# samivout/clair-torch

Hardware: AMD Instinct MI355X
Metric: MPix/s HDR-merged (+uncertainty) at N=32 4K RGB (higher is better)
Workload: dtype f32; 1 GPU; C2: 32-exposure 4096x4096x3 uint16 stack per GPU, merge+uncertainty (LINEAR ICRF 3x256, Gaussian weights, sigma: multiplier, float64 mean + float32 std out); global_image=4096x4096x3 in 1 row band(s)

## Files before the change

clair_torch_amd/_native.py:

```python
import ctypes
import os

from . import build as _build

DTYPE_U8, DTYPE_U16, DTYPE_F32 = 0, 1, 2
INTERP_LOOKUP, INTERP_LINEAR, INTERP_CATMULL, INTERP_NONE = 0, 1, 2, 3
STD_NONE, STD_CONSTANT, STD_MULTIPLIER, STD_EXPLICIT = 0, 1, 2, 3
WEIGHT_NONE, WEIGHT_GAUSS = 0, 1
LAYOUT_NCHW, LAYOUT_NHWC, LAYOUT_NHWC_BGR = 0, 1, 2
MERGE_FIRST_BATCH, MERGE_FINALIZE, MERGE_MEAN_OUT_F32, MERGE_F64_MOMENTS = 1, 2, 4, 8
MERGE_REFERENCE_ORDER, MERGE_CLOSED_FORM, MERGE_STD_HINT, MERGE_REQUIRE_ONE_LAUNCH, MERGE_OUT_AS_INPUT = 16, 32, 64, 128, 256
INGEST_AFFINE, INGEST_CLAMP, INGEST_MAX_STAGES, INGEST_MAX_CHANNELS = 0, 1, 4, 4
INGEST_AFFINE_DATA, EXTREMA_MIN, EXTREMA_MAX, EXTREMA_MAX_PREFIX = 2, 1, 2, 3
ERR_NO_GRADIENT_PATH = -4

ABI_VERSION = 3
EXPORTS = ("ct_abi_version", "ct_error_string", "ct_hdr_merge_batch", "ct_hdr_merge_batches", "ct_linearize_std", "ct_linearize_fwd",
           "ct_linearize_bwd", "ct_pair_residual_fwd", "ct_pair_residual_bwd", "ct_pair_residual_bwd_workspace", "ct_flatfield_sums",
           "ct_flatfield_apply", "ct_video_stats_batch", "ct_dark_field_blur", "ct_hdr_merge_kernel_name",
           "ct_merge_set_retry_counter", "ct_norm_constants", "ct_index_constants", "ct_pivot_index_constants",
           "ct_pivot_floor_constants", "ct_pivot_interval_constants", "ct_band_stats", "ct_band_stats_workspace",
           "ct_strided_downscale", "ct_export_cv", "ct_ingest_transform", "ct_ingest_extrema_workspace", "ct_ingest_extrema",
           "ct_ingest_transform_data", "ct_linearize_ingest")


class Geometry(ctypes.Structure):
    _fields_ = [("channels", ctypes.c_int32), ("h_tile", ctypes.c_int64), ("width", ctypes.c_int64),
                ("h_global", ctypes.c_int64), ("row_offset", ctypes.c_int64), ("image_stride", ctypes.c_int64),
                ("layout", ctypes.c_int32)]


class Icrf(ctypes.Structure):
    _fields_ = [("lut_dev", ctypes.c_void_p), ("n_points", ctypes.c_int32), ("interp", ctypes.c_int32)]


class PairParams(ctypes.Structure):
    _fields_ = [("lower", ctypes.c_float), ("upper", ctypes.c_float), ("weight_scale", ctypes.c_float),
                ("use_relative", ctypes.c_int32), ("use_uncertainty_weighting", ctypes.c_int32),
                ("std_mode", ctypes.c_int32), ("std_value", ctypes.c_float), ("pair_band", ctypes.c_int32)]


class IngestStage(ctypes.Structure):
    _fields_ = [("kind", ctypes.c_int32), ("sub", ctypes.c_float), ("div", ctypes.c_float), ("mul", ctypes.c_float),
                ("add", ctypes.c_float), ("lo", ctypes.c_float * 4), ("hi", ctypes.c_float * 4)]


class NativeLibraryError(RuntimeError):
    pass


_lib = None


def library_path():
    return _build.LIB_PATH


def load():
    global _lib
    if _lib is not None:
        return _lib
    path = library_path()
    if not os.path.exists(path):
        raise NativeLibraryError(
            f"{path} is missing: build it with `python -m clair_torch_amd.build` (hipcc, gfx950). "
            "clair_torch_amd has no CPU fallback for its kernels.")
    lib = ctypes.CDLL(path)
    vp, i32, i64, f32, u32 = ctypes.c_void_p, ctypes.c_int32, ctypes.c_int64, ctypes.c_float, ctypes.c_uint32
    gp, ip = ctypes.POINTER(Geometry), ctypes.POINTER(Icrf)
    lib.ct_abi_version.restype = i32
    lib.ct_error_string.restype = ctypes.c_char_p
    lib.ct_error_string.argtypes = [i32]
    lib.ct_hdr_merge_batch.restype = i32
    lib.ct_hdr_merge_batch.argtypes = [vp, i32, f32, i32, gp, vp, i32, f32, vp, ip, i32, vp, vp, vp, vp, vp, u32, vp]
    lib.ct_hdr_merge_batches.restype = i32
    lib.ct_hdr_merge_batches.argtypes = [vp, vp, vp, i32, i32, f32, gp, i32, f32, vp, ip, i32, vp, vp, vp, vp, vp, u32, vp]
    lib.ct_pivot_interval_constants.restype = i32
    lib.ct_pivot_interval_constants.argtypes = [f32, i32, i32, i32, ctypes.POINTER(f32)]
    lib.ct_linearize_std.restype = i32
    lib.ct_linearize_std.argtypes = [vp, i32, f32, i64, gp, vp, i32, f32, ip, vp, vp, vp]
    lib.ct_linearize_fwd.restype = i32
    lib.ct_linearize_fwd.argtypes = [vp, i64, gp, ip, vp, vp]
    lib.ct_linearize_bwd.restype = i32
    lib.ct_linearize_bwd.argtypes = [vp, vp, i64, gp, ip, vp, vp, vp]
    pp = ctypes.POINTER(PairParams)
    lib.ct_pair_residual_fwd.restype = i32
    lib.ct_pair_residual_fwd.argtypes = [vp, i32, f32, i32, gp, vp, ip, vp, vp, vp, i32, pp, i32, vp, vp, vp]
    lib.ct_pair_residual_bwd.restype = i32
    lib.ct_pair_residual_bwd.argtypes = [vp, i32, f32, i32, gp, vp, ip, vp, i32, vp, vp, vp, pp, vp, vp, vp, vp, i64, vp]
    lib.ct_pair_residual_bwd_workspace.restype = i64
    lib.ct_pair_residual_bwd_workspace.argtypes = [i32, i32, i32]
    lib.ct_hdr_merge_kernel_name.restype = ctypes.c_char_p
    lib.ct_hdr_merge_kernel_name.argtypes = [i32, f32, i32, i32, u32]
    lib.ct_merge_set_retry_counter.restype = None
    lib.ct_merge_set_retry_counter.argtypes = [vp]
    lib.ct_flatfield_sums.restype = i32
    lib.ct_flatfield_sums.argtypes = [vp, i32, vp, i32, i64, vp, vp]
    lib.ct_flatfield_apply.restype = i32
    lib.ct_flatfield_apply.argtypes = [vp, i32, i64, vp, i32, vp, vp, vp, vp, i32, i64, vp]
    lib.ct_dark_field_blur.restype = i32
    lib.ct_dark_field_blur.argtypes = [vp, i32, f32, i32, gp, vp, vp, i32, f32, vp, vp, i32, f32, f32, vp, vp, vp]
    lib.ct_band_stats_workspace.restype = i64
    lib.ct_band_stats_workspace.argtypes = [i32]
    lib.ct_band_stats.restype = i32
    lib.ct_band_stats.argtypes = [vp, vp, i32, i64, vp, i64, vp, vp]
    lib.ct_strided_downscale.restype = i32
    lib.ct_strided_downscale.argtypes = [vp, vp, i32, i64, i64, i64, i32, i32, vp]
    lib.ct_export_cv.restype = i32
    lib.ct_export_cv.argtypes = [vp, i32, vp, i32, i64, i32, i64, i32, vp]
    lib.ct_ingest_transform.restype = i32
    lib.ct_ingest_transform.argtypes = [vp, i32, i32, i64, i32, i64, ctypes.POINTER(IngestStage), i32, vp, vp]
    lib.ct_ingest_extrema_workspace.restype = i64
    lib.ct_ingest_extrema_workspace.argtypes = []
    lib.ct_ingest_extrema.restype = i32
    lib.ct_ingest_extrema.argtypes = [vp, i32, i32, i64, i32, i64, ctypes.POINTER(IngestStage), i32, i32, f32, f32, vp, i64, vp, vp]
    lib.ct_ingest_transform_data.restype = i32
    lib.ct_ingest_transform_data.argtypes = [vp, i32, i32, i64, i32, i64, ctypes.POINTER(IngestStage), i32, vp, vp, vp]
    lib.ct_linearize_ingest.restype = i32
    lib.ct_linearize_ingest.argtypes = [vp, i32, i64, gp, ctypes.POINTER(IngestStage), i32, vp, i32, f32, ip, vp, vp, vp]
    lib.ct_video_stats_batch.restype = i32
    lib.ct_video_stats_batch.argtypes = [vp, i32, f32, i32, gp, ip, f32, vp, vp, vp]
    if lib.ct_abi_version() != ABI_VERSION:
        raise NativeLibraryError(f"{path}: ABI version {lib.ct_abi_version()} != {ABI_VERSION}; rebuild the library")
    _lib = lib
    return lib


def check(rc, what):
    if rc == 0:
        return
    msg = load().ct_error_string(rc).decode()
    if rc == ERR_NO_GRADIENT_PATH:
        raise RuntimeError("element 0 of tensors does not require grad and does not have a grad_fn")
    if rc in (-1, -5):
        raise ValueError(f"{what}: {msg}")
    raise NativeLibraryError(f"{what}: {msg} (code {rc})")
```

clair_torch_amd/build.py:

```python
import os
import shutil
import subprocess
import sys
from concurrent.futures import ThreadPoolExecutor

HERE = os.path.dirname(os.path.abspath(__file__))
CSRC = os.path.join(HERE, "csrc")
LIB_DIR = os.path.join(HERE, "lib")
LIB_PATH = os.path.join(LIB_DIR, "libclair_hip.so")
OBJ_DIR = os.path.join(LIB_DIR, "obj")
SOURCES = ["ct_merge.hip", "ct_merge_multi.hip", "ct_merge_exact.hip", "ct_linearize.hip", "ct_pairs.hip", "ct_flatfield.hip", "ct_stats.hip", "ct_darkfield.hip", "ct_bandstats.hip",
           "ct_downscale.hip", "ct_export.hip", "ct_ingest.hip", "ct_extrema.hip", "ct_linearize_ingest.hip", "ct_api.cpp"]
HEADERS = ["ct_device.hpp", "ct_merge.hpp", "ct_merge_pivot.hpp", "ct_ingest_stages.hpp", os.path.join("..", "..", "include", "clair_hip.h")]
FLAGS = ["--offload-arch=gfx950", "-O3", "-std=c++17", "-fPIC", "-ffp-contract=off",
         "-fno-slp-vectorize", "-Wall", "-Wno-unused-function", "-Wno-pass-failed"]


def _hipcc():
    for cand in (os.environ.get("HIPCC"), shutil.which("hipcc"), "/opt/rocm/bin/hipcc"):
        if cand and os.path.exists(cand):
            return cand
    raise RuntimeError("hipcc not found (set HIPCC or install ROCm under /opt/rocm)")


def is_stale():
    if not os.path.exists(LIB_PATH):
        return True
    built = os.path.getmtime(LIB_PATH)
    deps = [os.path.join(CSRC, s) for s in SOURCES if os.path.exists(os.path.join(CSRC, s))]
    deps += [os.path.join(CSRC, h) for h in HEADERS]
    return any(os.path.getmtime(d) > built for d in deps)


def _object_is_stale(src, obj):
    if not os.path.exists(obj):
        return True
    built = os.path.getmtime(obj)
    return any(os.path.getmtime(d) > built for d in [src] + [os.path.join(CSRC, h) for h in HEADERS])


def build(force=False, verbose=False):
    if not force and not is_stale():
        return LIB_PATH
    os.makedirs(OBJ_DIR, exist_ok=True)
    hipcc = _hipcc()
    srcs = [os.path.join(CSRC, s) for s in SOURCES if os.path.exists(os.path.join(CSRC, s))]
    objs = [os.path.join(OBJ_DIR, os.path.basename(s) + ".o") for s in srcs]

    def compile_one(pair):
        src, obj = pair
        if not force and not _object_is_stale(src, obj):
            return
        cmd = [hipcc] + FLAGS + ["-c", "-o", obj, src]
        if verbose:
            print(" ".join(cmd), file=sys.stderr)
        subprocess.run(cmd, check=True)

    with ThreadPoolExecutor(max_workers=min(len(srcs), os.cpu_count() or 1)) as pool:
        list(pool.map(compile_one, zip(srcs, objs)))
    cmd = [hipcc, "--offload-arch=gfx950", "-shared", "-fPIC", "-o", LIB_PATH] + objs
    if verbose:
        print(" ".join(cmd), file=sys.stderr)
    subprocess.run(cmd, check=True)
    return LIB_PATH


if __name__ == "__main__":
    print(build(force="--force" in sys.argv, verbose=True))
```

clair_torch_amd/csrc/ct_api.cpp:

```cpp
#include <math.h>
#include <mutex>

#include "../../include/clair_hip.h"

extern "C" int ct_abi_version(void) { return CT_ABI_VERSION; }

extern "C" const char *ct_error_string(int code)
{
    switch (code) {
        case CT_OK: return "ok";
        case CT_ERR_INVALID_ARGUMENT: return "invalid argument";
        case CT_ERR_UNSUPPORTED: return "unsupported dtype or mode";
        case CT_ERR_LAUNCH: return "HIP kernel launch failed";
        case CT_ERR_NO_GRADIENT_PATH: return "no gradient path from the output to the image (reference raises RuntimeError)";
        case CT_ERR_TOO_LARGE: return "dimension too large for the kernel's indexing";
    }
    return "unknown error";
}

extern "C" int ct_norm_constants(float max_code, float *hi, float *lo)
{
    static std::mutex mu;
    static float cached_max = 0.0f, cached_hi = 0.0f, cached_lo = 0.0f;
    static int cached_rc = CT_ERR_UNSUPPORTED;
    if (!(max_code >= 1.0f) || max_code > 65535.0f || floorf(max_code) != max_code) return CT_ERR_UNSUPPORTED;
    std::lock_guard<std::mutex> lock(mu);
    if (cached_max != max_code) {
        const double rd = 1.0 / (double)max_code;
        const float h = (float)rd;
        const float l = (float)(rd - (double)h);
        int rc = CT_OK;
        for (int u = 0; u <= (int)max_code; ++u) {
            const float uf = (float)u;
            volatile float ref = uf / max_code;
            volatile float got = fmaf(uf, h, uf * l);
            if (ref != got) {
                rc = CT_ERR_UNSUPPORTED;
                break;
            }
        }
        cached_max = max_code;
        cached_hi = h;
        cached_lo = l;
        cached_rc = rc;
    }
    *hi = cached_hi;
    *lo = cached_lo;
    return cached_rc;
}

extern "C" int ct_index_constants(float max_code, int n_points, float *hi, float *lo)
{
    static std::mutex mu;
    static float cached_max = 0.0f, cached_hi = 0.0f, cached_lo = 0.0f;
    static int cached_L = 0, cached_rc = CT_ERR_UNSUPPORTED;
    if (!(max_code >= 1.0f) || max_code > 65535.0f || floorf(max_code) != max_code || n_points < 2)
        return CT_ERR_UNSUPPORTED;
    std::lock_guard<std::mutex> lock(mu);
    if (cached_max != max_code || cached_L != n_points) {
        const float top = (float)(n_points - 1);
        const double rd = (double)top / (double)max_code;
        const float h = (float)rd;
        const float l = (float)(rd - (double)h);
        int rc = CT_OK;
        for (int u = 0; u <= (int)max_code; ++u) {
            const float uf = (float)u;
            volatile float x = uf / max_code;
            volatile float s_ref = x * top;
            volatile float s_new = fmaf(uf, h, uf * l);
            if (floorf(s_ref) != floorf(s_new) || nearbyintf(s_ref) != nearbyintf(s_new) || s_new > top || s_new < 0.0f) {
                rc = CT_ERR_UNSUPPORTED;
                break;
            }
        }
        cached_max = max_code;
        cached_L = n_points;
        cached_hi = h;
        cached_lo = l;
        cached_rc = rc;
    }
    *hi = cached_hi;
    *lo = cached_lo;
    return cached_rc;
}

extern "C" int ct_pivot_index_constants(float max_code, int n_points, uint32_t *index_mul, float *step)
{
    static std::mutex mu;
    static float cached_max = 0.0f, cached_step = 0.0f;
    static uint32_t cached_mul = 0;
    static int cached_L = 0, cached_rc = CT_ERR_UNSUPPORTED;
    if (!(max_code >= 1.0f) || max_code > 65535.0f || floorf(max_code) != max_code || n_points < 2)
        return CT_ERR_UNSUPPORTED;
    std::lock_guard<std::mutex> lock(mu);
    if (cached_max != max_code || cached_L != n_points) {
        const int maxc = (int)max_code, top = n_points - 1;
        int rc = CT_OK;
        uint32_t mul = 0;
        float st = 0.0f;
        if (top > maxc || maxc % top != 0) {
            rc = CT_ERR_UNSUPPORTED;
        } else {
            const uint32_t istep = (uint32_t)(maxc / top);
            st = (float)istep;
            if (istep > 1) {
                const uint64_t m = ((1ull << 32) + istep - 1) / istep;
                if (m >= (1ull << 24)) rc = CT_ERR_UNSUPPORTED;
                mul = (uint32_t)m;
            }
            for (int u = 0; rc == CT_OK && u <= maxc; ++u) {
                volatile float x = (float)u / max_code;
                volatile float s_ref = x * (float)top;
                const uint32_t ref = (uint32_t)floorf(s_ref);
                const uint32_t got = istep > 1 ? (uint32_t)(((uint64_t)(uint32_t)u * mul) >> 32) : (uint32_t)u;
                if (ref != got || got > (uint32_t)top) rc = CT_ERR_UNSUPPORTED;
            }
        }
        cached_max = max_code;
        cached_L = n_points;
        cached_mul = mul;
        cached_step = st;
        cached_rc = rc;
    }
    *index_mul = cached_mul;
    *step = cached_step;
    return cached_rc;
}

extern "C" int ct_pivot_floor_constants(float max_code, int n_points, float *rcp_step)
{
    static std::mutex mu;
    static float cached_max = 0.0f, cached_rcp = 0.0f;
    static int cached_L = 0, cached_rc = CT_ERR_UNSUPPORTED;
    if (!(max_code >= 1.0f) || max_code > 65535.0f || floorf(max_code) != max_code || n_points < 2)
        return CT_ERR_UNSUPPORTED;
    if (n_points - 1 > (int)max_code || (int)max_code % (n_points - 1) != 0) return CT_ERR_UNSUPPORTED;
    const float step = (float)((int)max_code / (n_points - 1));
    std::lock_guard<std::mutex> lock(mu);
    if (cached_max != max_code || cached_L != n_points) {
        const int maxc = (int)max_code, top = n_points - 1;
        float r = (float)(1.0 / (double)step);
        if ((double)r < 1.0 / (double)step) r = nextafterf(r, 2.0f);
        int e = 0;
        const double m = frexp((double)r, &e);
        const uint64_t M = (uint64_t)ldexp(m, 24);
        const int shift = 24 - e;
        int rc = (shift >= 0 && shift < 63) ? CT_OK : CT_ERR_UNSUPPORTED;
        for (int u = 0; rc == CT_OK && u <= maxc; ++u) {
            volatile float x = (float)u / max_code;
            volatile float s_ref = x * (float)top;
            const uint64_t got = ((uint64_t)u * M) >> shift;
            if (got != (uint64_t)floorf(s_ref) || got > (uint64_t)top) rc = CT_ERR_UNSUPPORTED;
        }
        cached_max = max_code;
        cached_L = n_points;
        cached_rcp = r;
        cached_rc = rc;
    }
    *rcp_step = cached_rcp;
    return cached_rc;
}

extern "C" int ct_pivot_interval_constants(float max_code, int n_points, int lookup, int dtype_max, float *scale)
{
    struct Entry { float max_code; int n_points, lookup, dtype_max, rc; float scale; };
    static std::mutex mu;
    static Entry cache[8];
    static int used = 0, next = 0;
    if (!(max_code >= 1.0f) || max_code > 65535.0f || floorf(max_code) != max_code || n_points < 2 || dtype_max < (int)max_code ||
        dtype_max > 65535)
        return CT_ERR_UNSUPPORTED;
    std::lock_guard<std::mutex> lock(mu);
    for (int k = 0; k < used; ++k)
        if (cache[k].max_code == max_code && cache[k].n_points == n_points && cache[k].lookup == lookup && cache[k].dtype_max == dtype_max) {
            *scale = cache[k].scale;
            return cache[k].rc;
        }
    const int top = n_points - 1, last = lookup ? 2 * top : top;
    const double want = (double)(lookup ? 2 * top : top) / (double)max_code;
    float cand[4];
    cand[0] = (float)want;
    if ((double)cand[0] < want) cand[0] = nextafterf(cand[0], INFINITY);
    cand[1] = nextafterf(cand[0], INFINITY);
    cand[2] = nextafterf(cand[0], 0.0f);
    cand[3] = nextafterf(cand[2], 0.0f);
    int rc = CT_ERR_UNSUPPORTED;
    float found = 0.0f;
    for (int c = 0; c < 4 && rc != CT_OK; ++c) {
        const float r = cand[c];
        if (!((double)dtype_max * (double)r < 4194304.0)) continue;
        int e = 0;
        const double m = frexp((double)r, &e);
        const uint64_t M = (uint64_t)ldexp(m, 24);
        const int shift = 24 - e;
        if (shift < 0 || shift >= 63) continue;
        bool ok = true;
        for (int u = 0; ok && u <= dtype_max; ++u) {
            volatile float x = (float)u / max_code;
            volatile float s_ref = x * (float)top;
            float sc = s_ref < 0.0f ? 0.0f : (s_ref > (float)top ? (float)top : s_ref);
            uint64_t got = ((uint64_t)u * M) >> shift;
            if (got > (uint64_t)last) got = (uint64_t)last;
            if (lookup) {
                float rr = nearbyintf(s_ref);
                rr = rr < 0.0f ? 0.0f : (rr > (float)top ? (float)top : rr);
                ok = ((got + 1) >> 1) == (uint64_t)rr;
            } else {
                ok = got == (uint64_t)floorf(sc);
            }
        }
        if (ok) {
            rc = CT_OK;
            found = r;
        }
    }
    Entry &slot = cache[used < 8 ? used++ : (next++ % 8)];
    slot = Entry{max_code, n_points, lookup, dtype_max, rc, found};
    *scale = found;
    return rc;
}
```

clair_torch_amd/csrc/ct_merge.hip:

```cpp
#include "ct_merge_pivot.hpp"

namespace ct {

template <typename T, int V, int INTERP, int WEIGHT, int STD, bool FOLD, int PF = 2, bool PIVOT = true>
__global__ __launch_bounds__(kBlock) void merge_kernel(const MergeArgs a)
{
    extern __shared__ __align__(16) char lds[];
    constexpr bool kInt = sizeof(T) != 4;
    constexpr bool kRanged = kInt;
    constexpr bool kHasStd = STD != CT_STD_NONE;
    constexpr bool kGauss = WEIGHT == CT_WEIGHT_GAUSS;
    constexpr int kEntry = lut_entry_bytes(INTERP);
    static_assert(!FOLD || kInt, "FOLD is for integer codes");
    using Moment = std::conditional_t<PIVOT, float, double>;
    const int C = a.channels, L = a.n_points, B = a.batch;
    const int lut_bytes = INTERP == CT_INTERP_NONE ? 0 : C * L * kEntry;
    float *inv_t = reinterpret_cast<float *>(lds + lut_bytes);
    float *cq = inv_t + B;
    const float top = INTERP == CT_INTERP_NONE ? 1.0f : (float)(L - 1);
    const float kk = sqrtf(a.weight_scale * 1.4426950408889634f);
    const float K = -2.0f * a.weight_scale;

    stage_lut<INTERP, true>(lds, a.lut, C, L);
    for (int n = threadIdx.x; n < B; n += blockDim.x) {
        const float it = (float)(1.0 / a.exposure[n]);
        inv_t[n] = it;
        cq[n] = kGauss ? kk * top * it / K : top * it;
    }
    __syncthreads();

    const uint32_t vec = blockIdx.x * (uint32_t)kBlock + threadIdx.x;
    if (vec * (uint32_t)V >= a.q_count) return;
    const uint32_t q0 = a.q_begin + vec * (uint32_t)V;

    int row_off[V];
    if (a.tile.layout == CT_LAYOUT_NCHW) {
        int ch;
        uint32_t qg;
        a.tile.locate(q0, ch, qg);
        uint32_t off = q0 - (uint32_t)ch * a.tile.plane_local;
        int r = (int)(qg % (uint32_t)C);
        const int skip_mod = (int)(a.tile.chan_skip % (uint32_t)C);
#pragma unroll
        for (int e = 0; e < V; ++e) {
            row_off[e] = (INTERP == CT_INTERP_LOOKUP ? ch : r) * L * kEntry;
            int inc = 1;
            if (++off == a.tile.plane_local) {
                off = 0;
                ++ch;
                inc += skip_mod;
            }
            r += inc;
            r = r >= C ? r - C : r;
        }
    } else {
#pragma unroll
        for (int e = 0; e < V; ++e) {
            int ch;
            uint32_t qg;
            a.tile.locate(a.tile.planar_index(q0 + e), ch, qg);
            row_off[e] = lut_row<INTERP>(qg, ch, C) * L * kEntry;
        }
    }

    const T *src = static_cast<const T *>(a.stack) + q0;
    const float *ssrc = STD == CT_STD_EXPLICIT ? a.std_stack + q0 : nullptr;
    const float dk_mul = FOLD ? kk * a.inv_max_code : kk, dk_add = -0.5f * kk;
    const bool first = a.flags & CT_MERGE_FIRST_BATCH;
    const bool finalize = a.flags & CT_MERGE_FINALIZE;
    const bool keep_state = a.mean_state != nullptr;

    auto sample = [&](T code, int roff, float &px, float &lin, float &dfds) {
        float s;
        if constexpr (FOLD) {
            px = (float)code;
            s = __builtin_fmaf(px, a.index.hi, px * a.index.lo);
        } else {
            px = to_pixel<T>(code, a.norm);
            s = px * top;
        }
        if constexpr (INTERP == CT_INTERP_NONE) {
            lin = FOLD ? px * a.inv_max_code : px;
            dfds = 1.0f;
        } else if constexpr (INTERP == CT_INTERP_LOOKUP) {
            float r = rintf(s);
            r = kRanged ? fminf(r, top) : fminf(fmaxf(r, 0.0f), top);
            lin = reinterpret_cast<const float *>(lds + roff)[(int)r];
            dfds = 0.0f;
        } else {
            float pass = 1.0f;
            if constexpr (!kRanged) {
                pass = (s >= 0.0f && s <= top) ? 1.0f : 0.0f;
                s = fminf(fmaxf(s, 0.0f), top);
            } else {
                if constexpr (INTERP == CT_INTERP_CATMULL) pass = s <= top ? 1.0f : 0.0f;
                s = fminf(s, top);
            }
            const int i0 = (int)s;
            const float fr = __builtin_amdgcn_fractf(s);
            if constexpr (INTERP == CT_INTERP_LINEAR) {
                const float2 g = reinterpret_cast<const float2 *>(lds + roff)[i0];
                dfds = g.y;
                lin = __builtin_fmaf(dfds, fr, g.x);
                if constexpr (!kRanged) dfds *= pass;
            } else {
                const float4 g = reinterpret_cast<const float4 *>(lds + roff)[i0];
                const float t = fr, t2 = t * t, t3 = t2 * t;
                const float w0 = -0.5f * t3 + t2 - 0.5f * t, w1 = 1.5f * t3 - 2.5f * t2 + 1.0f;
                const float w2 = -1.5f * t3 + 2.0f * t2 + 0.5f * t, w3 = 0.5f * t3 - 0.5f * t2;
                lin = ((w0 * g.x + w1 * g.y) + w2 * g.z) + w3 * g.w;
                const float d0 = __builtin_fmaf(__builtin_fmaf(-1.5f, t, 2.0f), t, -0.5f);
                const float d2 = __builtin_fmaf(__builtin_fmaf(-4.5f, t, 4.0f), t, 0.5f);
                const float d3 = __builtin_fmaf(1.5f, t, -1.0f) * t;
                dfds = __builtin_fmaf(d0, g.x - g.y, __builtin_fmaf(d2, g.z - g.y, d3 * (g.w - g.y)));
                dfds *= pass;
            }
        }
    };

    [[maybe_unused]] float p[V];
    if constexpr (PIVOT) {
        if (first) {
            const int probe = B / 2;
            const Packet<T, V> pk = *reinterpret_cast<const Packet<T, V> *>(src + (int64_t)probe * a.image_stride);
            const float itp = inv_t[probe];
#pragma unroll
            for (int e = 0; e < V; ++e) {
                float px, lin, dfds;
                sample(pk.v[e], row_off[e], px, lin, dfds);
                p[e] = lin * itp;
            }
        } else {
#pragma unroll
            for (int e = 0; e < V; ++e) p[e] = (float)a.mean_state[a.out_index(q0 + e)];
        }
    }

    double mean_o[V];
    float std_o[V];
    for (int pass_no = 0;; ++pass_no) {
    float W[V], Swy[V];
    Moment Saa[V], Sab[V], Sbb[V];
#pragma unroll
    for (int e = 0; e < V; ++e) {
        W[e] = 0.0f;
        Swy[e] = 0.0f;
        Saa[e] = 0;
        Sab[e] = 0;
        Sbb[e] = 0;
    }

    Packet<T, V> ring[PF];
    Packet<float, V> sring[STD == CT_STD_EXPLICIT ? PF : 1];
#pragma unroll
    for (int k = 0; k < PF; ++k) {
        const int nn = k < B ? k : B - 1;
        ring[k] = *reinterpret_cast<const Packet<T, V> *>(src + (int64_t)nn * a.image_stride);
        if constexpr (STD == CT_STD_EXPLICIT)
            sring[k] = *reinterpret_cast<const Packet<float, V> *>(ssrc + (int64_t)nn * a.image_stride);
    }
#pragma unroll PF
    for (int n = 0; n < B; ++n) {
        const int nn = n + PF < B ? n + PF : B - 1;
        int64_t opaque_zero = 0;
        asm volatile("" : "+s"(opaque_zero));
        const int64_t eoff = (int64_t)nn * a.image_stride + opaque_zero;
        const Packet<T, V> incoming = *reinterpret_cast<const Packet<T, V> *>(src + eoff);
        Packet<float, V> sincoming;
        if constexpr (STD == CT_STD_EXPLICIT) sincoming = *reinterpret_cast<const Packet<float, V> *>(ssrc + eoff);
        const Packet<T, V> pk = ring[0];
        const Packet<float, V> sp = sring[0];
#pragma unroll
        for (int k = 0; k + 1 < PF; ++k) {
            ring[k] = ring[k + 1];
            if constexpr (STD == CT_STD_EXPLICIT) sring[k] = sring[k + 1];
        }
        ring[PF - 1] = incoming;
        if constexpr (STD == CT_STD_EXPLICIT) sring[PF - 1] = sincoming;
        const float it = inv_t[n];
        const float cqn = cq[n];
        float pxv[V], linv[V], dfv[V];
#pragma unroll
        for (int e = 0; e < V; ++e) sample(pk.v[e], row_off[e], pxv[e], linv[e], dfv[e]);
#pragma unroll
        for (int e = 0; e < V; ++e) {
            const float px = pxv[e], lin = linv[e], dfds = dfv[e];
            const float y = PIVOT ? __builtin_fmaf(lin, it, -p[e]) : lin * it;
            float sg = 1.0f;
            if constexpr (STD == CT_STD_EXPLICIT) sg = sp.v[e];
            if constexpr (STD == CT_STD_MULTIPLIER) sg = px;
            if constexpr (kGauss) {
                const float dk = __builtin_fmaf(px, dk_mul, dk_add);
                const float w = __builtin_amdgcn_exp2f(-dk * dk);
                W[e] += w;
                Swy[e] = __builtin_fmaf(w, y, Swy[e]);
                if constexpr (kHasStd) {
                    const float wu = (STD == CT_STD_CONSTANT) ? w : w * sg;
                    const float av = dk * wu;
                    float bv;
                    if constexpr (INTERP == CT_INTERP_LOOKUP)
                        bv = av * y;
                    else if constexpr (INTERP == CT_INTERP_NONE)
                        bv = __builtin_fmaf(av, y, wu * cqn);
                    else
                        bv = __builtin_fmaf(av, y, (wu * dfds) * cqn);
                    if constexpr (PIVOT) {
                        Saa[e] = __builtin_fmaf(av, av, Saa[e]);
                        Sab[e] = __builtin_fmaf(av, bv, Sab[e]);
                        Sbb[e] = __builtin_fmaf(bv, bv, Sbb[e]);
                    } else {
                        const double ad = (double)av, bd = (double)bv;
                        Saa[e] = __builtin_fma(ad, ad, Saa[e]);
                        Sab[e] = __builtin_fma(ad, bd, Sab[e]);
                        Sbb[e] = __builtin_fma(bd, bd, Sbb[e]);
                    }
                }
            } else {
                Swy[e] += y;
                if constexpr (kHasStd) {
                    const float bv = (INTERP == CT_INTERP_NONE ? sg : dfds * sg) * cqn;
                    if constexpr (PIVOT) {
                        Sbb[e] = __builtin_fmaf(bv, bv, Sbb[e]);
                    } else {
                        const double bd = (double)bv;
                        Sbb[e] = __builtin_fma(bd, bd, Sbb[e]);
                    }
                }
            }
        }
    }

    double fs = 1.0;
    if constexpr (kGauss) fs = (double)K / (double)kk;
    if constexpr (STD == CT_STD_CONSTANT) fs *= (double)a.std_value;
    if constexpr (STD == CT_STD_MULTIPLIER) fs *= (double)a.std_value * (FOLD ? (double)a.inv_max_code : 1.0);
    const double sv2 = fs * fs;
    bool any_bad = false;
    [[maybe_unused]] float mb_f[V];
    [[maybe_unused]] bool bad[V];
#pragma unroll
    for (int e = 0; e < V; ++e) {
        const uint32_t q = a.out_index(q0 + e);
        float Wb = W[e];
        if constexpr (!kGauss) Wb = (float)B;
        const float Df = Wb + 1e-6f;
        const float WA = first ? 0.0f : a.sumw_state[q];
        const double meanA = first ? 0.0 : a.mean_state[q];
        const float Wt = WA + Wb;
        const float frac = Wb / Wt;
        double mean;
        float var = 0.0f;
        if constexpr (PIVOT) {
            float r = __builtin_amdgcn_rcpf(Df);
            r = r * __builtin_fmaf(-Df, r, 2.0f);
            const float num = __builtin_fmaf(-p[e], 1e-6f, Swy[e]);
            float qd = num * r;
            qd = __builtin_fmaf(__builtin_fmaf(-qd, Df, num), r, qd);
            const double diff = ((double)p[e] - meanA) + (double)qd;
            mean = __builtin_fma((double)frac, diff, meanA);
            mb_f[e] = p[e] + qd;
            bad[e] = false;
            if constexpr (kHasStd) {
                const float gam = first ? 0.0f : (WA / (Wt * Wt)) * (float)diff;
                const float beta = frac * r;
                const float kap = __builtin_fmaf(-beta, qd, gam);
                const float t1 = beta * beta * Sbb[e];
                const float t2 = 2.0f * beta * kap * Sab[e];
                const float t3 = kap * kap * Saa[e];
                const float upd = (t1 + t2) + t3;
                if constexpr (kGauss) bad[e] = (t1 + fabsf(t2)) + t3 > kPivotCondLimit * upd;
                var = (first ? 0.0f : a.var_state[q]) + fmaxf(upd, 0.0f) * (float)sv2;
            }
            any_bad |= bad[e];
        } else {
            const double D = (double)Df;
            const double mb = (double)Swy[e] / D;
            mean = meanA + (double)frac * (mb - meanA);
            if constexpr (kHasStd) {
                const double beta = (double)frac / D;
                const double alpha = ((double)WA / ((double)Wt * (double)Wt)) * (mb - meanA) - beta * mb;
                const double upd = (alpha * alpha * (double)Saa[e] + 2.0 * alpha * beta * (double)Sab[e] + beta * beta * (double)Sbb[e]) * sv2;
                var = (first ? 0.0f : a.var_state[q]) + (float)upd;
            }
        }
        mean_o[e] = mean;
        std_o[e] = var;
        W[e] = Wt;
    }
    if constexpr (PIVOT) {
        if (pass_no == 0 && __any(any_bad)) {
#pragma unroll
            for (int e = 0; e < V; ++e) p[e] = bad[e] ? mb_f[e] : p[e];
            continue;
        }
    }
    if (keep_state) {
#pragma unroll
        for (int e = 0; e < V; ++e) {
            const uint32_t q = a.out_index(q0 + e);
            a.mean_state[q] = mean_o[e];
            a.sumw_state[q] = W[e];
            if constexpr (kHasStd) a.var_state[q] = std_o[e];
        }
    }
    break;
    }
#pragma unroll
    for (int e = 0; e < V; ++e) std_o[e] = __builtin_amdgcn_sqrtf(std_o[e]);
    if (finalize && a.tile.layout != CT_LAYOUT_NCHW && !(a.flags & CT_MERGE_OUT_AS_INPUT)) {
#pragma unroll
        for (int e = 0; e < V; ++e) {
            const uint32_t q = a.tile.planar_index(q0 + e);
            if (a.flags & CT_MERGE_MEAN_OUT_F32)
                static_cast<float *>(a.mean_out)[q] = (float)mean_o[e];
            else
                static_cast<double *>(a.mean_out)[q] = mean_o[e];
            if constexpr (kHasStd) a.std_out[q] = std_o[e];
        }
    } else if (finalize) {
        if (a.flags & CT_MERGE_MEAN_OUT_F32) {
            Packet<float, V> o;
#pragma unroll
            for (int e = 0; e < V; ++e) o.v[e] = (float)mean_o[e];
            store_stream(reinterpret_cast<Packet<float, V> *>(static_cast<float *>(a.mean_out) + q0), o);
        } else {
            Packet<double, V> o;
#pragma unroll
            for (int e = 0; e < V; ++e) o.v[e] = mean_o[e];
            store_stream(reinterpret_cast<Packet<double, V> *>(static_cast<double *>(a.mean_out) + q0), o);
        }
        if constexpr (kHasStd) {
            Packet<float, V> o;
#pragma unroll
            for (int e = 0; e < V; ++e) o.v[e] = std_o[e];
            store_stream(reinterpret_cast<Packet<float, V> *>(a.std_out + q0), o);
        }
    }
}

template <typename T, int V, int INTERP, int WEIGHT, int STD, bool CLAMP>
static int launch_pivot(const MergeArgs &a, PivotArgs x, hipStream_t stream)
{
    if (a.q_count == 0) return CT_OK;
    if constexpr (INTERP == CT_INTERP_LOOKUP && WEIGHT == CT_WEIGHT_NONE && STD != CT_STD_NONE) {
        return CT_ERR_NO_GRADIENT_PATH;
    } else {
        x.n_tiles = (a.q_count + (uint32_t)(kBlock * V) - 1) / (uint32_t)(kBlock * V);
        size_t lds = pivot_lds_bytes(a, x, INTERP);
        x.rgb252 = 0;
        if constexpr (V == 4) {
            auto aligned16 = [](const void *p) { return (reinterpret_cast<uintptr_t>(p) % 16) == 0; };
            if (a.tile.layout != CT_LAYOUT_NCHW && !(a.flags & CT_MERGE_OUT_AS_INPUT) && a.channels == 3 && a.tile.plane_local % 4 == 0 && !a.mean_state &&
                (a.flags & CT_MERGE_FINALIZE) && !(a.flags & CT_MERGE_MEAN_OUT_F32) && a.q_begin == 0 &&
                a.q_count == 3u * a.tile.plane_local && aligned16(a.mean_out) && aligned16(a.std_out)) {
                x.rgb252 = 1;
                lds = (lds + 15) & ~(size_t)15;
                x.stage_off = (uint32_t)lds;
                lds += 4 * 3072;
            }
        }
        if (lds > 160 * 1024) return CT_ERR_TOO_LARGE;
        if constexpr (V == 4) {
            if (x.rgb252)
                return (a.flags & CT_MERGE_FIRST_BATCH)
                           ? launch_pivot_grid<merge_pivot_kernel<T, V, INTERP, WEIGHT, STD, true, CLAMP, false, true>>(a, x, lds, stream)
                           : CT_ERR_INVALID_ARGUMENT;
        }
        return (a.flags & CT_MERGE_FIRST_BATCH)
                   ? launch_pivot_grid<merge_pivot_kernel<T, V, INTERP, WEIGHT, STD, true, CLAMP>>(a, x, lds, stream)
                   : launch_pivot_grid<merge_pivot_kernel<T, V, INTERP, WEIGHT, STD, false, CLAMP>>(a, x, lds, stream);
    }
}

template <typename T, int V>
static int dispatch_pivot(const MergeArgs &a, const PivotArgs &x, int interp, int weight_mode, int std_mode, bool clamp, hipStream_t s)
{
    return with_merge_modes(interp, weight_mode, std_mode, [&](auto I, auto W, auto S) {
        if constexpr (I == CT_INTERP_NONE) {
            return launch_pivot<T, V, I, W, S, false>(a, x, s);
        } else if constexpr (V == 1) {
            return launch_pivot<T, V, I, W, S, true>(a, x, s);
        } else if constexpr (sizeof(T) == 2) {
            return clamp ? launch_pivot<T, V, I, W, S, true>(a, x, s) : launch_pivot<T, V, I, W, S, false>(a, x, s);
        } else {
            return launch_pivot<T, V, I, W, S, false>(a, x, s);
        }
    });
}

template <typename T, int V, int INTERP, int WEIGHT, int STD>
static int launch_one(const MergeArgs &a, hipStream_t stream, bool fold)
{
    if (a.q_count == 0) return CT_OK;
    const uint32_t vecs = a.q_count / V;
    const uint32_t grid = (vecs + kBlock - 1) / kBlock;
    const size_t lds = (INTERP == CT_INTERP_NONE ? 0 : (size_t)a.channels * a.n_points * lut_entry_bytes(INTERP)) +
                       2 * sizeof(float) * (size_t)a.batch;
    if (lds > 160 * 1024) return CT_ERR_TOO_LARGE;
    const bool f64 = a.flags & CT_MERGE_F64_MOMENTS;
    if constexpr (sizeof(T) != 4) {
        if (fold && f64)
            hipLaunchKernelGGL((merge_kernel<T, V, INTERP, WEIGHT, STD, true, 2, false>), dim3(grid), dim3(kBlock), lds, stream, a);
        else if (fold)
            hipLaunchKernelGGL((merge_kernel<T, V, INTERP, WEIGHT, STD, true, 2, true>), dim3(grid), dim3(kBlock), lds, stream, a);
        else if (f64)
            hipLaunchKernelGGL((merge_kernel<T, V, INTERP, WEIGHT, STD, false, 2, false>), dim3(grid), dim3(kBlock), lds, stream, a);
        else
            hipLaunchKernelGGL((merge_kernel<T, V, INTERP, WEIGHT, STD, false, 2, true>), dim3(grid), dim3(kBlock), lds, stream, a);
    } else if (f64) {
        hipLaunchKernelGGL((merge_kernel<T, V, INTERP, WEIGHT, STD, false, 2, false>), dim3(grid), dim3(kBlock), lds, stream, a);
    } else {
        hipLaunchKernelGGL((merge_kernel<T, V, INTERP, WEIGHT, STD, false, 2, true>), dim3(grid), dim3(kBlock), lds, stream, a);
    }
    return hipGetLastError() == hipSuccess ? CT_OK : CT_ERR_LAUNCH;
}

template <typename T, int V>
static int dispatch_generic(const MergeArgs &a, int interp, int weight_mode, int std_mode, hipStream_t s, bool fold)
{
    return with_merge_modes(interp, weight_mode, std_mode, [&](auto I, auto W, auto S) { return launch_one<T, V, I, W, S>(a, s, fold); });
}


template <typename T>
struct VecWidth {
    static constexpr int value = sizeof(T) == 1 ? 8 : 4;
};

static bool packets_aligned(const MergeArgs &a, size_t elem_bytes, int V, bool with_state)
{
    auto ok = [V](const void *p, size_t bytes) { return reinterpret_cast<uintptr_t>(p) % (bytes * V) == 0; };
    return ok(a.stack, elem_bytes) && a.image_stride % V == 0 && ok(a.std_stack, 4) && ok(a.mean_out, 8) && ok(a.std_out, 4) &&
           (!with_state || (ok(a.mean_state, 8) && ok(a.sumw_state, 4) && ok(a.var_state, 4)));
}

template <typename T>
static int merge_typed(MergeArgs a, uint32_t Q, int interp, int weight_mode, int std_mode, hipStream_t s, bool fold,
                       const PivotArgs *pivot = nullptr, bool pivot_clamp = false)
{
    constexpr int V = VecWidth<T>::value;
    int rc = CT_OK;
    if constexpr (sizeof(T) != 4) {
        if (pivot) {
            const uint32_t q_pv = packets_aligned(a, sizeof(T), kPivotV, false) ? (Q / kPivotV) * kPivotV : 0;
            a.q_begin = 0;
            a.q_count = q_pv;
            if (q_pv) rc = dispatch_pivot<T, kPivotV>(a, *pivot, interp, weight_mode, std_mode, pivot_clamp, s);
            a.q_begin = q_pv;
            a.q_count = Q - q_pv;
            if (rc == CT_OK && q_pv < Q) rc = dispatch_pivot<T, 1>(a, *pivot, interp, weight_mode, std_mode, pivot_clamp, s);
            return rc;
        }
    }
    const uint32_t q_vec = packets_aligned(a, sizeof(T), V, true) ? (Q / V) * V : 0;
    a.q_begin = 0;
    a.q_count = q_vec;
    if (q_vec) rc = dispatch_generic<T, V>(a, interp, weight_mode, std_mode, s, fold);
    a.q_begin = q_vec;
    a.q_count = Q - q_vec;
    if (rc == CT_OK && q_vec < Q) rc = dispatch_generic<T, 1>(a, interp, weight_mode, std_mode, s, fold);
    return rc;
}

}

extern "C" int ct_norm_constants(float max_code, float *hi, float *lo);
extern "C" int ct_index_constants(float max_code, int n_points, float *hi, float *lo);
extern "C" int ct_pivot_interval_constants(float max_code, int n_points, int lookup, int dtype_max, float *scale);

static unsigned long long *g_merge_retry_counter = nullptr;
extern "C" void ct_merge_set_retry_counter(unsigned long long *counter_dev) { g_merge_retry_counter = counter_dev; }

enum class MergeRoute {
    ReferenceOrder,
    Pivot,
    Generic
};

static MergeRoute merge_route(int32_t dtype, float max_code, int interp, int n_points, int std_mode, uint32_t flags,
                              ct::PivotArgs *px, bool *clamp)
{
    if (flags & CT_MERGE_REFERENCE_ORDER) return MergeRoute::ReferenceOrder;
    if ((interp == CT_INTERP_CATMULL || interp == CT_INTERP_LOOKUP) && std_mode != CT_STD_NONE &&
        !(flags & (CT_MERGE_CLOSED_FORM | CT_MERGE_F64_MOMENTS)))
        return MergeRoute::ReferenceOrder;
    if ((dtype != CT_DTYPE_U8 && dtype != CT_DTYPE_U16) || (flags & CT_MERGE_F64_MOMENTS)) return MergeRoute::Generic;
    const int dtype_max = dtype == CT_DTYPE_U8 ? 255 : 65535;
    if (!(max_code >= 1.0f) || max_code > (float)dtype_max || floorf(max_code) != max_code) return MergeRoute::Generic;
    if (interp < CT_INTERP_LOOKUP || interp > CT_INTERP_NONE) return MergeRoute::Generic;
    const bool lookup = interp == CT_INTERP_LOOKUP;
    *clamp = interp != CT_INTERP_NONE && max_code < (float)dtype_max;
    px->step = 1.0f;
    px->index_rcp = 1.0f;
    px->max_code = max_code;
    px->n_entries = 0;
    px->tf_max = ct::kFloorMagic;
    if (interp == CT_INTERP_NONE) return MergeRoute::Pivot;
    if (*clamp && dtype == CT_DTYPE_U8) return MergeRoute::Generic;
    if (ct_pivot_interval_constants(max_code, n_points, lookup, dtype_max, &px->index_rcp) != CT_OK) return MergeRoute::Generic;
    px->step = (float)((double)max_code / (double)(n_points - 1));
    px->n_entries = lookup ? 2u * (uint32_t)n_points : (uint32_t)n_points;
    px->tf_max = ct::kFloorMagic + (float)(lookup ? 2 * (n_points - 1) : n_points - 1);
    return MergeRoute::Pivot;
}

extern "C" const char *ct_hdr_merge_kernel_name(int32_t dtype, float max_code, int32_t interp, int32_t n_points,
                                                uint32_t flags)
{
    ct::PivotArgs px{};
    bool clamp = false;
    switch (merge_route(dtype, max_code, interp, n_points, (flags & CT_MERGE_STD_HINT) ? CT_STD_CONSTANT : CT_STD_NONE, flags, &px, &clamp)) {
        case MergeRoute::ReferenceOrder:
            return "ct::merge_reference_order_kernel (the reference's float32 autograd order, two passes, float64 exp and divisions)";
        case MergeRoute::Pivot:
            return (flags & CT_MERGE_FIRST_BATCH)
                       ? "ct::merge_pivot_kernel (float32 moments about a per-pixel pivot, persistent workgroups, 4 codes per "
                         "thread through typed buffer loads, 7 wavefronts per SIMD, first batch)"
                       : "ct::merge_pivot_kernel (float32 moments about the running mean, persistent workgroups, 4 codes per "
                         "thread, streaming state)";
        case MergeRoute::Generic: break;
    }
    if (flags & CT_MERGE_F64_MOMENTS)
        return dtype == CT_DTYPE_F32 ? "ct::merge_kernel (float64 moments, float32 pixels, 4 per thread)"
                                     : "ct::merge_kernel (float64 moments, integer codes)";
    return dtype == CT_DTYPE_F32 ? "ct::merge_kernel (float32 moments about a per-pixel pivot, float32 pixels, 4 per thread)"
                                 : "ct::merge_kernel (float32 moments about a per-pixel pivot, integer codes through the float LUT coordinate)";
}

struct MergeCall {
    const ct_geometry *geom;
    int32_t std_mode;
    float std_value;
    const double *exposure;
    const ct_icrf *icrf;
    int32_t weight_mode;
    double *mean_state;
    float *sumw_state, *var_state;
    void *mean_out;
    float *std_out;
    uint32_t flags;
    bool has_state() const { return mean_state && sumw_state && (std_mode == CT_STD_NONE || var_state); }
    bool state_ok() const { return has_state() || ((flags & CT_MERGE_FIRST_BATCH) && (flags & CT_MERGE_FINALIZE)); }
    bool positive_shape() const { return geom->channels > 0 && geom->h_tile > 0 && geom->width > 0; }
    bool no_gradient_path() const { return std_mode != CT_STD_NONE && icrf->interp == CT_INTERP_LOOKUP && weight_mode == CT_WEIGHT_NONE; }
    int64_t local_elements() const { return geom->h_tile * geom->width * geom->channels; }
};

static int validate_merge(const MergeCall &c)
{
    const ct_geometry *geom = c.geom;
    if (!geom || !c.icrf || !c.exposure) return CT_ERR_INVALID_ARGUMENT;
    if (!c.positive_shape() || geom->h_global < geom->h_tile || geom->row_offset < 0 || geom->row_offset + geom->h_tile > geom->h_global)
        return CT_ERR_INVALID_ARGUMENT;
    if (geom->layout < CT_LAYOUT_NCHW || geom->layout > CT_LAYOUT_NHWC_BGR) return CT_ERR_INVALID_ARGUMENT;
    const int interp = c.icrf->interp;
    if (interp < CT_INTERP_LOOKUP || interp > CT_INTERP_NONE) return CT_ERR_INVALID_ARGUMENT;
    if (interp != CT_INTERP_NONE && (!c.icrf->lut_dev || c.icrf->n_points < 2)) return CT_ERR_INVALID_ARGUMENT;
    if (c.std_mode < CT_STD_NONE || c.std_mode > CT_STD_EXPLICIT) return CT_ERR_INVALID_ARGUMENT;
    if (c.weight_mode != CT_WEIGHT_NONE && c.weight_mode != CT_WEIGHT_GAUSS) return CT_ERR_INVALID_ARGUMENT;
    if (c.no_gradient_path()) return CT_ERR_NO_GRADIENT_PATH;
    if (!c.state_ok()) return CT_ERR_INVALID_ARGUMENT;
    if ((c.flags & CT_MERGE_FINALIZE) && (!c.mean_out || (c.std_mode != CT_STD_NONE && !c.std_out))) return CT_ERR_INVALID_ARGUMENT;
    if (geom->h_global * geom->width * geom->channels >= (int64_t)1 << 31) return CT_ERR_TOO_LARGE;
    if (geom->image_stride < c.local_elements()) return CT_ERR_INVALID_ARGUMENT;
    return CT_OK;
}

static ct::MergeArgs fill_merge_args(const MergeCall &c, const void *stack, const float *std_stack, int32_t batch)
{
    const ct_geometry *geom = c.geom;
    const int64_t plane_g = geom->h_global * geom->width, plane_l = geom->h_tile * geom->width;
    const bool has_state = c.has_state();
    ct::MergeArgs a{};
    a.stack = stack;
    a.std_stack = c.std_mode == CT_STD_EXPLICIT ? std_stack : nullptr;
    a.exposure = c.exposure;
    a.lut = c.icrf->lut_dev;
    a.mean_state = has_state ? c.mean_state : nullptr;
    a.sumw_state = has_state ? c.sumw_state : nullptr;
    a.var_state = has_state ? c.var_state : nullptr;
    a.mean_out = c.mean_out;
    a.std_out = c.std_out;
    a.image_stride = geom->image_stride;
    a.tile.plane_local = (uint32_t)plane_l;
    a.tile.chan_skip = (uint32_t)(plane_g - plane_l);
    a.tile.base = (uint32_t)(geom->row_offset * geom->width);
    a.tile.layout = (uint32_t)geom->layout;
    a.tile.channels = (uint32_t)geom->channels;
    a.batch = batch;
    a.channels = geom->channels;
    a.n_points = c.icrf->interp == CT_INTERP_NONE ? 2 : c.icrf->n_points;
    a.std_value = c.std_value;
    a.weight_scale = 30.0f;
    a.inv_max_code = 1.0f;
    a.flags = c.flags;
    return a;
}

extern "C" int ct_hdr_merge_batch(const void *stack_dev, int32_t dtype, float max_code, int32_t batch,
                                  const ct_geometry *geom, const float *std_dev, int32_t std_mode, float std_value,
                                  const double *exposure_dev, const ct_icrf *icrf, int32_t weight_mode,
                                  double *mean_state_dev, float *sumw_state_dev, float *var_state_dev,
                                  void *mean_out_dev, float *std_out_dev, uint32_t flags, void *stream)
{
    using namespace ct;
    const MergeCall c{geom, std_mode, std_value, exposure_dev, icrf, weight_mode, mean_state_dev, sumw_state_dev, var_state_dev,
                      mean_out_dev, std_out_dev, flags};
    if (!stack_dev || batch <= 0 || (std_mode == CT_STD_EXPLICIT && !std_dev)) return CT_ERR_INVALID_ARGUMENT;
    if (const int rc = validate_merge(c); rc != CT_OK) return rc;
    MergeArgs a = fill_merge_args(c, stack_dev, std_dev, batch);
    const uint32_t Ql = (uint32_t)c.local_elements();
    const int interp = icrf->interp;
    hipStream_t s = static_cast<hipStream_t>(stream);
    PivotArgs px{};
    bool clamp = false;
    const MergeRoute route = merge_route(dtype, max_code, interp, a.n_points, std_mode, flags, &px, &clamp);
    if (dtype != CT_DTYPE_F32 && ct_norm_constants(max_code, &a.norm.hi, &a.norm.lo) != CT_OK) return CT_ERR_UNSUPPORTED;
    if (route == MergeRoute::ReferenceOrder) return merge_reference_order(a, dtype, Ql, interp, weight_mode, std_mode, s);
    if (dtype == CT_DTYPE_F32) return merge_typed<float>(a, Ql, interp, weight_mode, std_mode, s, false);
    if (dtype != CT_DTYPE_U8 && dtype != CT_DTYPE_U16) return CT_ERR_UNSUPPORTED;
    const bool fold = ct_index_constants(max_code, a.n_points, &a.index.hi, &a.index.lo) == CT_OK;
    a.inv_max_code = (float)(1.0 / (double)max_code);
    px.probe = batch / 2;
    px.retry_count = g_merge_retry_counter;
    const PivotArgs *pivot = route == MergeRoute::Pivot ? &px : nullptr;
    return dtype == CT_DTYPE_U8 ? merge_typed<uint8_t>(a, Ql, interp, weight_mode, std_mode, s, fold, pivot, clamp)
                                : merge_typed<uint16_t>(a, Ql, interp, weight_mode, std_mode, s, fold, pivot, clamp);
}

extern "C" int ct_hdr_merge_batches(const void *const *stack_devs, const float *const *std_devs, const int32_t *batch_sizes,
                                    int32_t n_batches, int32_t dtype, float max_code, const ct_geometry *geom, int32_t std_mode,
                                    float std_value, const double *exposure_dev, const ct_icrf *icrf, int32_t weight_mode,
                                    double *mean_state_dev, float *sumw_state_dev, float *var_state_dev, void *mean_out_dev,
                                    float *std_out_dev, uint32_t flags, void *stream)
{
    using namespace ct;
    if (!stack_devs || !batch_sizes || n_batches <= 0 || !geom || !icrf || !exposure_dev) return CT_ERR_INVALID_ARGUMENT;
    if (std_mode == CT_STD_EXPLICIT && !std_devs) return CT_ERR_INVALID_ARGUMENT;
    int64_t total = 0;
    for (int b = 0; b < n_batches; ++b) {
        if (!stack_devs[b] || batch_sizes[b] <= 0 || (std_mode == CT_STD_EXPLICIT && !std_devs[b])) return CT_ERR_INVALID_ARGUMENT;
        total += batch_sizes[b];
    }
    const MergeCall c{geom, std_mode, std_value, exposure_dev, icrf, weight_mode, mean_state_dev, sumw_state_dev, var_state_dev,
                      mean_out_dev, std_out_dev, flags};
    const int valid = validate_merge(c);
    const int interp = icrf->interp;
    const int64_t Ql = c.local_elements();
    hipStream_t s = static_cast<hipStream_t>(stream);
    MergeArgs a = fill_merge_args(c, stack_devs[0], std_mode == CT_STD_EXPLICIT ? std_devs[0] : nullptr, (int32_t)total);
    PivotArgs px{};
    bool clamp = false;
    const MergeRoute route = merge_route(dtype, max_code, interp, a.n_points, std_mode, flags, &px, &clamp);

    if (route == MergeRoute::ReferenceOrder && valid == CT_OK && n_batches >= 2 && n_batches <= kMaxMergeBatches && total <= 65536 &&
        (dtype == CT_DTYPE_U8 || dtype == CT_DTYPE_U16 || dtype == CT_DTYPE_F32)) {
        if (dtype != CT_DTYPE_F32 && ct_norm_constants(max_code, &a.norm.hi, &a.norm.lo) != CT_OK) return CT_ERR_UNSUPPORTED;
        MergeBatches mb{};
        mb.n_batches = n_batches;
        for (int b = 0; b < n_batches; ++b) {
            mb.batch_size[b] = batch_sizes[b];
            mb.batch_ptr[b] = stack_devs[b];
            mb.std_ptr[b] = std_mode == CT_STD_EXPLICIT ? std_devs[b] : nullptr;
        }
        return merge_reference_order(a, dtype, (uint32_t)Ql, interp, weight_mode, std_mode, s, &mb);
    }
    bool fast = route == MergeRoute::Pivot && n_batches >= 2 && n_batches <= kMaxMultiBatches && total <= 0x7fffffff && c.state_ok() &&
                c.positive_shape() && !c.no_gradient_path() && Ql % kPivotV == 0;
    for (int b = 0; fast && b < n_batches; ++b) {
        a.stack = stack_devs[b];
        a.std_stack = std_mode == CT_STD_EXPLICIT ? std_devs[b] : nullptr;
        fast = packets_aligned(a, dtype == CT_DTYPE_U8 ? 1 : 2, kPivotV, false);
    }
    if (fast) {
        if (valid != CT_OK) return valid;
        if (ct_norm_constants(max_code, &a.norm.hi, &a.norm.lo) != CT_OK) return CT_ERR_UNSUPPORTED;
        a.stack = stack_devs[0];
        a.std_stack = std_mode == CT_STD_EXPLICIT ? std_devs[0] : nullptr;
        a.q_begin = 0;
        a.q_count = (uint32_t)Ql;
        a.inv_max_code = (float)(1.0 / (double)max_code);
        px.n_batches = n_batches;
        px.fresh = (flags & CT_MERGE_FIRST_BATCH) ? 1 : 0;
        px.probe = batch_sizes[0] / 2;
        px.retry_count = g_merge_retry_counter;
        for (int b = 0; b < n_batches; ++b) {
            px.batch_size[b] = batch_sizes[b];
            px.batch_ptr[b] = stack_devs[b];
            px.std_ptr[b] = std_mode == CT_STD_EXPLICIT ? std_devs[b] : nullptr;
        }
        return merge_pivot_multi(a, px, dtype, clamp, interp, weight_mode, std_mode, s);
    }
    if (flags & CT_MERGE_REQUIRE_ONE_LAUNCH) return CT_ERR_UNSUPPORTED;
    if (n_batches > 1 && !c.has_state()) return CT_ERR_INVALID_ARGUMENT;
    const bool first = flags & CT_MERGE_FIRST_BATCH, finalize = flags & CT_MERGE_FINALIZE;
    int64_t n0 = 0;
    for (int b = 0; b < n_batches; ++b) {
        const uint32_t f = (flags & ~(CT_MERGE_FIRST_BATCH | CT_MERGE_FINALIZE)) | ((first && b == 0) ? CT_MERGE_FIRST_BATCH : 0u) |
                           ((finalize && b == n_batches - 1) ? CT_MERGE_FINALIZE : 0u);
        const int rc = ct_hdr_merge_batch(stack_devs[b], dtype, max_code, batch_sizes[b], geom, std_devs ? std_devs[b] : nullptr,
                                          std_mode, std_value, exposure_dev + n0, icrf, weight_mode, mean_state_dev,
                                          sumw_state_dev, var_state_dev, mean_out_dev, std_out_dev, f, stream);
        if (rc != CT_OK) return rc;
        n0 += batch_sizes[b];
    }
    return CT_OK;
}
```

clair_torch_amd/csrc/ct_merge_pivot.hpp:

```cpp
#pragma once
#include "ct_merge.hpp"
#include <type_traits>

namespace ct {


constexpr int kStackLoadAux = 0;
template <typename P>
__device__ __forceinline__ P load_buffer(uint64_t base, uint32_t offset)
{
    const __amdgpu_buffer_rsrc_t rsrc =
        __builtin_amdgcn_make_buffer_rsrc(reinterpret_cast<void *>(base), 0, 0xffffffff, 0x00020000 );
    P out;
    if constexpr (sizeof(P) == 1) {
        const uint8_t v = __builtin_amdgcn_raw_buffer_load_b8(rsrc, offset, 0, kStackLoadAux);
        __builtin_memcpy(&out, &v, sizeof(P));
    } else if constexpr (sizeof(P) == 2) {
        const uint16_t v = __builtin_amdgcn_raw_buffer_load_b16(rsrc, offset, 0, kStackLoadAux);
        __builtin_memcpy(&out, &v, sizeof(P));
    } else if constexpr (sizeof(P) == 4) {
        const uint32_t v = __builtin_amdgcn_raw_buffer_load_b32(rsrc, offset, 0, kStackLoadAux);
        __builtin_memcpy(&out, &v, sizeof(P));
    } else if constexpr (sizeof(P) == 8) {
        typedef uint32_t vec_t __attribute__((ext_vector_type(2)));
        const vec_t v = __builtin_amdgcn_raw_buffer_load_b64(rsrc, offset, 0, kStackLoadAux);
        __builtin_memcpy(&out, &v, sizeof(P));
    } else {
        static_assert(sizeof(P) == 16, "packets are at most 16 bytes");
        typedef uint32_t vec_t __attribute__((ext_vector_type(4)));
        const vec_t v = __builtin_amdgcn_raw_buffer_load_b128(rsrc, offset, 0, kStackLoadAux);
        __builtin_memcpy(&out, &v, sizeof(P));
    }
    return out;
}

template <typename T, int V>
__device__ __forceinline__ Packet<float, V> load_codes_as_float(uint64_t base, uint32_t offset)
{
    Packet<float, V> out;
    load_codes_as_float<T, V, kStackLoadAux>(base, offset, out.v);
    return out;
}


template <int N, int I = 0, typename F>
__device__ __forceinline__ void static_for(F &&f)
{
    if constexpr (I < N) {
        f(std::integral_constant<int, I>{});
        static_for<N, I + 1>(f);
    }
}

struct PivotArgs {
    uint32_t index_mul;
    float step;
    uint32_t n_tiles;
    int32_t probe;
    float index_rcp;
    float max_code;
    float tf_max;
    uint32_t n_entries;
    unsigned long long *retry_count;
    int32_t n_batches;
    int32_t fresh;
    int32_t batch_size[16];
    const void *batch_ptr[16];
    const float *std_ptr[16];
    int32_t rgb252;
    uint32_t stage_off;
};
constexpr int kMaxMultiBatches = 16;
constexpr int kPivotV = 4;

constexpr int kPivotDepth = 2;
constexpr float kRoughLimit = 64.0f;


constexpr int kRgb252Waves = 6;
template <typename T, int V, int INTERP, int WEIGHT, int STD, bool FIRST, bool CLAMP = false, bool MULTI = false, bool RGB252 = false>
__global__ __launch_bounds__(kBlock)
__attribute__((amdgpu_waves_per_eu(FIRST && V <= 4 && STD != CT_STD_EXPLICIT ? (RGB252 ? kRgb252Waves : 7) : 4, 8)))
void merge_pivot_kernel(const MergeArgs a, const PivotArgs x)
{
    static_assert(!MULTI || !FIRST, "MULTI carries state");
    static_assert(!RGB252 || (V == 4 && FIRST && !MULTI), "RGB252: single-batch packets");
    extern __shared__ __align__(16) char lds[];
    static_assert(sizeof(T) != 4, "raw integer codes only");
    constexpr bool kLut = INTERP != CT_INTERP_NONE;
    constexpr bool kLookup = INTERP == CT_INTERP_LOOKUP;
    constexpr bool kCat = INTERP == CT_INTERP_CATMULL;
    constexpr bool kHasStd = STD != CT_STD_NONE;
    constexpr bool kGauss = WEIGHT == CT_WEIGHT_GAUSS;
    using CodePk = Packet<float, V>;
    const int C = a.channels, L = a.n_points, B = a.batch;
    constexpr int kEntryShift = kCat ? 4 : 3;
    const int E = kLut ? (int)x.n_entries : 0;
    const int lut_bytes = C * E * (1 << kEntryShift);
    float2 *expo = reinterpret_cast<float2 *>(lds + lut_bytes);
    const float kk = sqrtf(a.weight_scale * 1.4426950408889634f);
    const float dk_mul = kk * a.inv_max_code, dk_add = -0.5f * kk;
    const float K = -2.0f * a.weight_scale;
    const float max_code = kLut ? x.max_code : 1.0f;
    const float ce = kGauss ? max_code * kk / K : max_code;

    bool rough = false;
    if constexpr (kLookup) {
        const int total = C * E;
        for (int k = threadIdx.x; k < total; k += kBlock) {
            const int r = k / E, j = k - r * E;
            const int idx = (j + 1) >> 1;
            reinterpret_cast<float2 *>(lds)[k] = make_float2(a.lut[(size_t)r * L + (idx < L ? idx : L - 1)], 0.0f);
        }
    } else if constexpr (kCat) {
        const int total = C * L;
        const double st = (double)x.step;
        for (int k = threadIdx.x; k < total; k += kBlock) {
            const int r = k / L, i = k - r * L;
            const float *row = a.lut + (size_t)r * L;
            const double p0 = row[i > 0 ? i - 1 : 0], p1 = row[i], p2 = row[i + 1 < L ? i + 1 : L - 1], p3 = row[i + 2 < L ? i + 2 : L - 1];
            const double c1 = 0.5 * (p2 - p0), b1 = 0.5 * (2.0 * p0 - 5.0 * p1 + 4.0 * p2 - p3), a1 = 0.5 * (-p0 + 3.0 * p1 - 3.0 * p2 + p3);
            reinterpret_cast<float4 *>(lds)[k] = make_float4((float)p1, (float)(c1 / st), (float)(b1 / (st * st)), (float)(a1 / (st * st * st)));
        }
    } else if constexpr (kLut) {
        const int total = C * L;
        const double stepd = (double)x.max_code / (double)(L - 1);
        bool viol = false;
        for (int k = threadIdx.x; k < total; k += kBlock) {
            const int r = k / L, i = k - r * L;
            const float *row = a.lut + (size_t)r * L;
            const float g0 = row[i], g1 = row[i + 1 < L ? i + 1 : L - 1];
            const float slope = (g1 - g0) / x.step;
            const float A = (float)((double)g0 - (double)slope * ((double)i * stepd));
            viol |= !(fabsf(A) <= kRoughLimit * fmaxf(fmaxf(fabsf(g0), fabsf(g1)), 1e-30f));
        }
        rough = __syncthreads_or(viol);
        for (int k = threadIdx.x; k < total; k += kBlock) {
            const int r = k / L, i = k - r * L;
            const float *row = a.lut + (size_t)r * L;
            const float g0 = row[i], g1 = row[i + 1 < L ? i + 1 : L - 1];
            const float slope = (g1 - g0) / x.step;
            const float A = (float)((double)g0 - (double)slope * ((double)i * stepd));
            reinterpret_cast<float2 *>(lds)[k] = make_float2(rough ? g0 : A, slope);
        }
    }
    for (int n = threadIdx.x; n < B; n += kBlock) {
        const float it = (float)(1.0 / a.exposure[n]);
        expo[n] = make_float2(it, ce * it);
    }
    __syncthreads();

    const bool finalize = a.flags & CT_MERGE_FINALIZE;
    const bool keep_state = a.mean_state != nullptr;
    const bool planar = a.tile.layout == CT_LAYOUT_NCHW;
    const bool planar_out = planar || (a.flags & CT_MERGE_OUT_AS_INPUT);
    float fsf = 1.0f;
    if constexpr (kGauss) fsf = K / kk;
    if constexpr (STD == CT_STD_CONSTANT) fsf *= a.std_value;
    if constexpr (STD == CT_STD_MULTIPLIER) fsf *= a.std_value * a.inv_max_code;
    const float sv2 = fsf * fsf;
    [[maybe_unused]] const float index_rcp = x.index_rcp;
    [[maybe_unused]] float floor_magic = kFloorMagic;
    asm volatile("" : "+v"(floor_magic));

    constexpr bool rgb252 = RGB252;
    for (uint32_t tile = blockIdx.x; tile < x.n_tiles; tile += gridDim.x) {
        const uint32_t vec = tile * (uint32_t)kBlock + threadIdx.x;
        if (vec * (uint32_t)V >= a.q_count) continue;
        const uint32_t q0 = a.q_begin + vec * (uint32_t)V;

        int row_off[V];
        if constexpr (kLut) {
            if (planar) {
                int ch = 0;
                for (int c = 1; c < C; ++c) ch += q0 >= (uint32_t)c * a.tile.plane_local ? 1 : 0;
                const uint32_t qg = q0 + (uint32_t)ch * a.tile.chan_skip + a.tile.base;
                uint32_t off = q0 - (uint32_t)ch * a.tile.plane_local;
                int r = C == 3 ? (int)(qg % 3u) : (int)(qg % (uint32_t)C);
                const int skip_mod = (int)(a.tile.chan_skip % (uint32_t)C);
#pragma unroll
                for (int e = 0; e < V; ++e) {
                    row_off[e] = (kLookup ? ch : r) * E * 8;
                    int inc = 1;
                    if (++off == a.tile.plane_local) {
                        off = 0;
                        ++ch;
                        inc += skip_mod;
                    }
                    r += inc;
                    r = r >= C ? r - C : r;
                }
            } else if (C == 3) {
                const uint32_t plane_g = a.tile.plane_local + a.tile.chan_skip;
#pragma unroll
                for (int e = 0; e < V; ++e) {
                    uint32_t c, pixel;
                    a.tile.interleaved3(q0 + e, c, pixel);
                    const uint32_t qg = c * plane_g + a.tile.base + pixel;
                    row_off[e] = (int)(kLookup ? c : qg % 3u) * E * 8;
                }
            } else {
#pragma unroll
                for (int e = 0; e < V; ++e) {
                    int ch;
                    uint32_t qg;
                    a.tile.locate(a.tile.planar_index(q0 + e), ch, qg);
                    row_off[e] = (kLookup ? ch : (int)(qg % (uint32_t)C)) * E * 8;
                }
            }
        } else {
#pragma unroll
            for (int e = 0; e < V; ++e) row_off[e] = 0;
        }
        [[maybe_unused]] uint32_t rowc[V];
        if constexpr (kLut) {
#pragma unroll
            for (int e = 0; e < V; ++e) rowc[e] = lds_row_constant<kEntryShift>(row_off[e] << (kEntryShift - 3));
        }

        const uint32_t voff = q0 * (uint32_t)sizeof(T), svoff = q0 * 4u;
        auto planar_of = [&](uint32_t m) -> uint32_t {
            if (planar_out) return m;
            if (C == 3) {
                uint32_t c, pixel;
                a.tile.interleaved3(m, c, pixel);
                return c * a.tile.plane_local + pixel;
            }
            return a.tile.planar_index(m);
        };

        constexpr int VS = FIRST ? 1 : V;
        float p[V], WA[VS], varA[VS];
        double meanA[VS];
        [[maybe_unused]] auto probe_pivot = [&](uint64_t stack_base) {
            const Packet<float, V> pk = load_codes_as_float<T, V>(
                stack_base + (uint64_t)((int64_t)x.probe * a.image_stride * (int64_t)sizeof(T)), voff);
            const float itp = expo[x.probe].x;
            float tf[V];
            if constexpr (kLut) floor_index_bits<V>(pk.v, index_rcp, floor_magic, tf);
            if constexpr (kLut && CLAMP) {
#pragma unroll
                for (int e = 0; e < V; ++e) tf[e] = fminf(tf[e], x.tf_max);
            }
#pragma unroll
            for (int e = 0; e < V; ++e) {
                const float px = pk.v[e];
                float lin = px * a.inv_max_code;
                if constexpr (kCat) {
                    const float4 g = *reinterpret_cast<const float4 *>(lds + lds_entry_address<kEntryShift>(tf[e], rowc[e]));
                    float o = __builtin_fmaf(tf[e] - floor_magic, -x.step, px);
                    if constexpr (CLAMP) o = px > x.max_code ? 0.0f : o;
                    lin = __builtin_fmaf(__builtin_fmaf(__builtin_fmaf(g.w, o, g.z), o, g.y), o, g.x);
                } else if constexpr (kLut) {
                    const float2 g = *reinterpret_cast<const float2 *>(lds + lds_entry_address<kEntryShift>(tf[e], rowc[e]));
                    lin = __builtin_fmaf(g.y, rough ? __builtin_fmaf(tf[e] - floor_magic, -x.step, px) : px, g.x);
                }
                p[e] = lin * itp;
            }
        };
        if constexpr (FIRST) {
            probe_pivot(reinterpret_cast<uint64_t>(a.stack));
        } else {
            bool fresh = false;
            if constexpr (MULTI) fresh = x.fresh != 0;
            if (fresh) {
                if constexpr (MULTI) {
#pragma unroll
                    for (int e = 0; e < V; ++e) {
                        meanA[e] = 0.0;
                        WA[e] = 0.0f;
                        varA[e] = 0.0f;
                    }
                    probe_pivot(reinterpret_cast<uint64_t>(x.batch_ptr[0]));
                }
            } else {
#pragma unroll
                for (int e = 0; e < V; ++e) {
                    const uint32_t q = planar_of(q0 + e);
                    meanA[e] = a.mean_state[q];
                    WA[e] = a.sumw_state[q];
                    if constexpr (kHasStd) varA[e] = a.var_state[q];
                    p[e] = (float)meanA[e];
                }
            }
        }

        double mean_o[V];
        float var_o[V], Wt_o[V];
        const int n_batches = MULTI ? x.n_batches : 1;
        int n0 = 0;
        for (int bi = 0; bi < n_batches; ++bi) {
        const int Bb = MULTI ? x.batch_size[bi] : B;
        const uint64_t batch_base = MULTI ? reinterpret_cast<uint64_t>(x.batch_ptr[bi]) : reinterpret_cast<uint64_t>(a.stack);
        [[maybe_unused]] const uint64_t batch_std_base = MULTI ? reinterpret_cast<uint64_t>(x.std_ptr[bi]) : reinterpret_cast<uint64_t>(a.std_stack);
        for (int pass = 0;; ++pass) {
            float W[V], Swy[V], Saa[V], Sac[V], Scc[V];
#pragma unroll
            for (int e = 0; e < V; ++e) W[e] = Swy[e] = Saa[e] = Sac[e] = Scc[e] = 0.0f;

            auto run_batch = [&](auto rough_c, auto moments_c) {
            constexpr bool kRough = decltype(rough_c)::value;
            constexpr bool kMoments = decltype(moments_c)::value;
            auto reduce = [&](const CodePk &pk, const Packet<float, V> &sp, uint32_t expo_adr) {
                const float2 ex = *reinterpret_cast<const float2 *>(lds + expo_adr);
                const float it = ex.x, cqn = ex.y;
                float pxv[V], ga[V], gs[V];
                [[maybe_unused]] float pxl[V];
                [[maybe_unused]] float dkv[V], wv[V];
                [[maybe_unused]] float tf[V];
#pragma unroll
                for (int e = 0; e < V; ++e) pxv[e] = pk.v[e];
                if constexpr (kLut) floor_index_bits<V>(pxv, index_rcp, floor_magic, tf);
                if constexpr (kLut && CLAMP) {
#pragma unroll
                    for (int e = 0; e < V; ++e) tf[e] = fminf(tf[e], x.tf_max);
                }
                static_for<V>([&](auto ec) {
                    constexpr int e = decltype(ec)::value;
                    if constexpr (kCat) {
                        const float4 g = *reinterpret_cast<const float4 *>(lds + lds_entry_address<4>(tf[e], rowc[e]));
                        float o = __builtin_fmaf(tf[e] - floor_magic, -x.step, pxv[e]);
                        [[maybe_unused]] bool above = false;
                        if constexpr (CLAMP) {
                            above = pxv[e] > x.max_code;
                            o = above ? 0.0f : o;
                        }
                        ga[e] = __builtin_fmaf(__builtin_fmaf(__builtin_fmaf(g.w, o, g.z), o, g.y), o, g.x);
                        gs[e] = 0.0f;
                        if constexpr (kHasStd) {
                            gs[e] = __builtin_fmaf(__builtin_fmaf(3.0f * g.w, o, g.z + g.z), o, g.y);
                            if constexpr (CLAMP) gs[e] = above ? 0.0f : gs[e];
                        }
                    } else if constexpr (kLut) {
                        const float2 g = *reinterpret_cast<const float2 *>(lds + lds_entry_address(tf[e], rowc[e]));
                        ga[e] = g.x;
                        gs[e] = g.y;
                        if constexpr (kRough) pxl[e] = __builtin_fmaf(tf[e] - floor_magic, -x.step, pxv[e]);
                    }
                    if constexpr (kGauss) {
                        dkv[e] = __builtin_fmaf(pxv[e], dk_mul, dk_add);
                        wv[e] = __builtin_amdgcn_exp2f(-dkv[e] * dkv[e]);
                    }
                });
                if constexpr (kGauss) {
#pragma unroll
                    for (int e = 0; e < V; ++e) asm volatile("" : "+v"(wv[e]));
                }
#pragma unroll
                for (int e = 0; e < V; ++e) {
                    const float px = pxv[e];
                    const float lin = (kLookup || kCat) ? ga[e] : kLut ? __builtin_fmaf(gs[e], kRough ? pxl[e] : px, ga[e]) : px * a.inv_max_code;
                    const float yd = __builtin_fmaf(lin, it, -p[e]);
                    if constexpr (kGauss) {
                        const float dk = dkv[e], w = wv[e];
                        W[e] += w;
                        Swy[e] = __builtin_fmaf(w, yd, Swy[e]);
                        if constexpr (kHasStd && kMoments) {
                            float wu = w;
                            if constexpr (STD == CT_STD_MULTIPLIER) wu = w * px;
                            if constexpr (STD == CT_STD_EXPLICIT) wu = w * sp.v[e];
                            const float av = dk * wu;
                            float cv;
                            if constexpr (kLookup) {
                                cv = av * yd;
                            } else {
                                const float ev = kLut ? (wu * gs[e]) * cqn : wu * cqn;
                                cv = __builtin_fmaf(av, yd, ev);
                            }
                            Saa[e] = __builtin_fmaf(av, av, Saa[e]);
                            Sac[e] = __builtin_fmaf(av, cv, Sac[e]);
                            Scc[e] = __builtin_fmaf(cv, cv, Scc[e]);
                        }
                    } else {
                        Swy[e] += yd;
                        if constexpr (kHasStd) {
                            float ev = kLut ? gs[e] * cqn : cqn;
                            if constexpr (STD == CT_STD_MULTIPLIER) ev *= px;
                            if constexpr (STD == CT_STD_EXPLICIT) ev *= sp.v[e];
                            Scc[e] = __builtin_fmaf(ev, ev, Scc[e]);
                        }
                    }
                }
            };

            auto fetch = [&](int n, CodePk &pk, Packet<float, V> &sp) {
                const int nn = n < Bb ? n : Bb - 1;
                uint64_t base = batch_base + (uint64_t)((int64_t)nn * a.image_stride * (int64_t)sizeof(T));
                asm volatile("" : "+s"(base));
                pk = load_codes_as_float<T, V>(base, voff);
                if constexpr (STD == CT_STD_EXPLICIT) {
                    uint64_t sbase = batch_std_base + (uint64_t)((int64_t)nn * a.image_stride * 4);
                    asm volatile("" : "+s"(sbase));
                    sp = load_buffer<Packet<float, V>>(sbase, svoff);
                }
            };
            constexpr int kRing = kPivotDepth + 1;
            CodePk ring[kRing];
            Packet<float, V> sring[STD == CT_STD_EXPLICIT ? kRing : 1];
            static_for<kPivotDepth>([&](auto jc) {
                constexpr int j = decltype(jc)::value;
                fetch(j, ring[j], sring[STD == CT_STD_EXPLICIT ? j : 0]);
            });
            uint32_t expo_adr = (uint32_t)lut_bytes + 8u * (uint32_t)n0;
            for (int n = 0; n < Bb; n += kRing) {
                static_for<kRing>([&](auto jc) {
                    constexpr int j = decltype(jc)::value, slot = (j + kPivotDepth) % kRing;
                    fetch(n + j + kPivotDepth, ring[slot], sring[STD == CT_STD_EXPLICIT ? slot : 0]);
                    if (j == 0 || n + j < Bb) reduce(ring[j], sring[STD == CT_STD_EXPLICIT ? j : 0], expo_adr + 8u * j);
                });
                expo_adr += 8u * kRing;
            }
            };
            constexpr bool kMeanFirst = kLookup && kHasStd;
            if constexpr (kMeanFirst) {
                if (pass == 0)
                    run_batch(std::false_type{}, std::false_type{});
                else
                    run_batch(std::false_type{}, std::true_type{});
            } else {
                if (rough)
                    run_batch(std::true_type{}, std::true_type{});
                else
                    run_batch(std::false_type{}, std::true_type{});
            }

            bool bad[V];
            float mb_f[V];
#pragma unroll
            for (int e = 0; e < V; ++e) {
                const float Wb = kGauss ? W[e] : (float)Bb;
                const float Df = Wb + 1e-6f;
                const float r = __builtin_amdgcn_rcpf(Df);
                const float num = __builtin_fmaf(-p[e], 1e-6f, Swy[e]);
                float q = num * r;
                q = __builtin_fmaf(__builtin_fmaf(-q, Df, num), r, q);
                float Wt = Wb, frac = 1.0f, var = 0.0f, gam = 0.0f;
                bad[e] = false;
                if constexpr (FIRST) {
                    mean_o[e] = (double)p[e] + (double)q;
                } else {
                    Wt = WA[e] + Wb;
                    const float rw = __builtin_amdgcn_rcpf(Wt);
                    frac = WA[e] == 0.0f ? 1.0f : Wb * rw;
                    const double diff = ((double)p[e] - meanA[e]) + (double)q;
                    mean_o[e] = __builtin_fma((double)frac, diff, meanA[e]);
                    gam = ((WA[e] * rw) * rw) * (float)diff;
                    var = varA[e];
                }
                Wt_o[e] = Wt;
                mb_f[e] = p[e] + q;
                if constexpr (kHasStd) {
                    const float beta = frac * r;
                    const float kap = __builtin_fmaf(-beta, q, gam);
                    const float bk = beta * kap;
                    const float S = __builtin_fmaf(kap * kap, Saa[e], (beta * beta) * Scc[e]);
                    const float upd = __builtin_fmaf(bk + bk, Sac[e], S);
                    if constexpr (kGauss) bad[e] = upd * (0.5f * (kPivotCondLimit + 1.0f)) < S;
                    if constexpr (kMeanFirst) bad[e] = bad[e] || pass == 0;
                    var += fmaxf(upd, 0.0f) * sv2;
                }
                var_o[e] = var;
            }
            bool any_bad = false;
#pragma unroll
            for (int e = 0; e < V; ++e) any_bad |= bad[e];
            if (pass == 1 || !__any(any_bad)) break;
            if (x.retry_count && (threadIdx.x & 63) == 0) atomicAdd(x.retry_count, 1ull);
#pragma unroll
            for (int e = 0; e < V; ++e) p[e] = bad[e] ? mb_f[e] : p[e];
        }
        if constexpr (MULTI) {
#pragma unroll
            for (int e = 0; e < V; ++e) {
                meanA[e] = mean_o[e];
                WA[e] = Wt_o[e];
                varA[e] = var_o[e];
                p[e] = (float)mean_o[e];
            }
            n0 += Bb;
        }
        }

        if (keep_state) {
#pragma unroll
            for (int e = 0; e < V; ++e) {
                const uint32_t q = planar_of(q0 + e);
                a.mean_state[q] = mean_o[e];
                a.sumw_state[q] = Wt_o[e];
                if constexpr (kHasStd) a.var_state[q] = var_o[e];
            }
        }
        if (finalize && rgb252) {
            if constexpr (RGB252) {
                const uint32_t tile_first = tile * (uint32_t)(kBlock * V);
                const bool tile_full = tile_first + (uint32_t)(kBlock * V) <= a.q_count;
                float sdv[4];
#pragma unroll
                for (int e = 0; e < 4; ++e) sdv[e] = kHasStd ? __builtin_amdgcn_sqrtf(var_o[e]) : 0.0f;
                if (tile_full) {
                    char *stage = lds + x.stage_off;
                    double *sm = reinterpret_cast<double *>(stage);
                    float *ss = reinterpret_cast<float *>(stage + 8192);
                    typedef double d2 __attribute__((ext_vector_type(2)));
                    typedef float f4 __attribute__((ext_vector_type(4)));
                    __syncthreads();
                    d2 m01 = {mean_o[0], mean_o[1]}, m23 = {mean_o[2], mean_o[3]};
                    *reinterpret_cast<d2 *>(sm + 4u * threadIdx.x) = m01;
                    *reinterpret_cast<d2 *>(sm + 4u * threadIdx.x + 2) = m23;
                    if constexpr (kHasStd) {
                        f4 sv = {sdv[0], sdv[1], sdv[2], sdv[3]};
                        *reinterpret_cast<f4 *>(ss + 4u * threadIdx.x) = sv;
                    }
                    __syncthreads();
                    const uint32_t g_first = (tile_first + 11u) / 12u, g_end = (tile_first + (uint32_t)(kBlock * V)) / 12u;
#pragma unroll
                    for (int e = 0; e < 4; ++e) {
                        const uint32_t m = q0 + (uint32_t)e - a.q_begin;
                        if (m < 12u * g_first || m >= 12u * g_end) {
                            const uint32_t q = planar_of(q0 + e);
                            static_cast<double *>(a.mean_out)[q] = mean_o[e];
                            if constexpr (kHasStd) a.std_out[q] = sdv[e];
                        }
                    }
                    const uint32_t n_groups = g_end - g_first;
                    const uint32_t c = (threadIdx.x >= n_groups ? 1u : 0u) + (threadIdx.x >= 2u * n_groups ? 1u : 0u);
                    const uint32_t tri = threadIdx.x - c * n_groups;
                    if (threadIdx.x < 3u * n_groups) {
                        const uint32_t g = g_first + tri;
                        const uint32_t cm = a.tile.layout == CT_LAYOUT_NHWC_BGR ? 2u - c : c;
                        const uint32_t local = 12u * g - tile_first + cm;
                        Packet<double, 4> mo;
                        Packet<float, 4> so;
#pragma unroll
                        for (int j = 0; j < 4; ++j) {
                            mo.v[j] = sm[local + 3u * (uint32_t)j];
                            if constexpr (kHasStd) so.v[j] = ss[local + 3u * (uint32_t)j];
                        }
                        const size_t dst = (size_t)c * a.tile.plane_local + 4u * (size_t)g;
                        store_stream(reinterpret_cast<Packet<double, 4> *>(static_cast<double *>(a.mean_out) + dst), mo);
                        if constexpr (kHasStd) store_stream(reinterpret_cast<Packet<float, 4> *>(a.std_out + dst), so);
                    }
                } else {
#pragma unroll
                    for (int e = 0; e < 4; ++e) {
                        const uint32_t q = planar_of(q0 + e);
                        static_cast<double *>(a.mean_out)[q] = mean_o[e];
                        if constexpr (kHasStd) a.std_out[q] = sdv[e];
                    }
                }
            }
        } else if (finalize && !planar_out) {
#pragma unroll
            for (int e = 0; e < V; ++e) {
                const uint32_t q = planar_of(q0 + e);
                if (a.flags & CT_MERGE_MEAN_OUT_F32)
                    static_cast<float *>(a.mean_out)[q] = (float)mean_o[e];
                else
                    static_cast<double *>(a.mean_out)[q] = mean_o[e];
                if constexpr (kHasStd) a.std_out[q] = __builtin_amdgcn_sqrtf(var_o[e]);
            }
        } else if (finalize) {
            if (a.flags & CT_MERGE_MEAN_OUT_F32) {
                Packet<float, V> o;
#pragma unroll
                for (int e = 0; e < V; ++e) o.v[e] = (float)mean_o[e];
                store_stream(reinterpret_cast<Packet<float, V> *>(static_cast<float *>(a.mean_out) + q0), o);
            } else {
                Packet<double, V> o;
#pragma unroll
                for (int e = 0; e < V; ++e) o.v[e] = mean_o[e];
                store_stream(reinterpret_cast<Packet<double, V> *>(static_cast<double *>(a.mean_out) + q0), o);
            }
            if constexpr (kHasStd) {
                Packet<float, V> o;
#pragma unroll
                for (int e = 0; e < V; ++e) o.v[e] = __builtin_amdgcn_sqrtf(var_o[e]);
                store_stream(reinterpret_cast<Packet<float, V> *>(a.std_out + q0), o);
            }
        }
    }
}

template <typename KernelT>
static int pivot_blocks_per_cu(KernelT kernel, size_t lds)
{
    int n = 0;
    if (hipOccupancyMaxActiveBlocksPerMultiprocessor(&n, kernel, kBlock, lds) != hipSuccess || n < 1) n = 1;
    return n < 8 ? n : 8;
}

template <auto kernel>
static int launch_pivot_grid(const MergeArgs &a, const PivotArgs &x, size_t lds, hipStream_t stream)
{
    static int per_cu = 0;
    static size_t per_cu_lds = 0;
    if (per_cu == 0 || lds > per_cu_lds) {
        per_cu = pivot_blocks_per_cu(kernel, lds);
        per_cu_lds = lds;
    }
    uint32_t grid = (uint32_t)(compute_units() * per_cu);
    if (grid > x.n_tiles) grid = x.n_tiles;
    hipLaunchKernelGGL(kernel, dim3(grid), dim3(kBlock), lds, stream, a, x);
    return hipGetLastError() == hipSuccess ? CT_OK : CT_ERR_LAUNCH;
}

static size_t pivot_lds_bytes(const MergeArgs &a, const PivotArgs &x, int interp)
{
    const size_t table = interp == CT_INTERP_NONE ? 0 : (size_t)a.channels * x.n_entries * (interp == CT_INTERP_CATMULL ? 16 : 8);
    return table + 2 * sizeof(float) * (size_t)a.batch;
}

template <int... VALUES, typename F>
static int with_enum(int value, F &&f)
{
    int rc = CT_ERR_INVALID_ARGUMENT;
    (void)((value == VALUES ? (rc = f(std::integral_constant<int, VALUES>{}), true) : false) || ...);
    return rc;
}

template <typename F>
static int with_merge_modes(int interp, int weight_mode, int std_mode, F &&f)
{
    return with_enum<CT_INTERP_LOOKUP, CT_INTERP_LINEAR, CT_INTERP_CATMULL, CT_INTERP_NONE>(interp, [&](auto I) {
        return with_enum<CT_WEIGHT_NONE, CT_WEIGHT_GAUSS>(weight_mode, [&](auto W) {
            return with_enum<CT_STD_NONE, CT_STD_CONSTANT, CT_STD_MULTIPLIER, CT_STD_EXPLICIT>(std_mode, [&](auto S) { return f(I, W, S); });
        });
    });
}

int merge_pivot_multi(const MergeArgs &a, const PivotArgs &px, int dtype, bool clamp, int interp, int weight_mode, int std_mode,
                      hipStream_t s);

}
```

clair_torch_amd/ops.py:

```python
import ctypes
from dataclasses import dataclass
from typing import Optional

import torch

from . import _native as nv

_INTERP = {"lookup": nv.INTERP_LOOKUP, "linear": nv.INTERP_LINEAR, "catmull": nv.INTERP_CATMULL, None: nv.INTERP_NONE}
_STD = {"none": nv.STD_NONE, "constant": nv.STD_CONSTANT, "multiplier": nv.STD_MULTIPLIER, "explicit": nv.STD_EXPLICIT}
_DTYPE = {torch.uint8: nv.DTYPE_U8, torch.uint16: nv.DTYPE_U16, torch.float32: nv.DTYPE_F32}
_LAYOUT = {"nchw": nv.LAYOUT_NCHW, "nhwc": nv.LAYOUT_NHWC, "nhwc_bgr": nv.LAYOUT_NHWC_BGR}


@dataclass
class TileGeometry:
    h_global: int
    row_offset: int = 0


def _require_device(t: torch.Tensor, name: str):
    if not isinstance(t, torch.Tensor):
        raise TypeError(f"{name} must be a torch.Tensor, got {type(t)}")
    if not t.is_cuda:
        raise RuntimeError(f"{name} is on {t.device}: clair_torch_amd kernels run on MI355X (cuda/ROCm) tensors only; "
                           "there is no CPU path in this package")


def _ptr(t: Optional[torch.Tensor]):
    return None if t is None else ctypes.c_void_p(t.data_ptr())


def _stream(device):
    return ctypes.c_void_p(torch.cuda.current_stream(device).cuda_stream)


def _chw(stack: torch.Tensor, layout: str):
    if layout not in _LAYOUT:
        raise ValueError(f"unknown layout {layout!r} (nchw, nhwc, nhwc_bgr)")
    if layout == "nchw":
        return stack.shape[1], stack.shape[2], stack.shape[3]
    return stack.shape[3], stack.shape[1], stack.shape[2]


def _out_shape(stack: torch.Tensor, layout: str, out_layout: str):
    if out_layout not in ("planar", "input"):
        raise ValueError(f"unknown out_layout {out_layout!r} (planar, input)")
    return tuple(stack.shape[1:]) if out_layout == "input" else tuple(_chw(stack, layout))


def _geometry(stack: torch.Tensor, tile: Optional[TileGeometry], layout: str = "nchw") -> nv.Geometry:
    c, h, w = _chw(stack, layout)
    hg, r0 = (h, 0) if tile is None else (tile.h_global, tile.row_offset)
    if r0 < 0 or r0 + h > hg:
        raise ValueError(f"tile rows [{r0}, {r0 + h}) do not fit a global height of {hg}")
    return nv.Geometry(channels=c, h_tile=h, width=w, h_global=hg, row_offset=r0, image_stride=stack.stride(0),
                       layout=_LAYOUT[layout])


def _check_stack(stack: torch.Tensor, name="stack"):
    _require_device(stack, name)
    if stack.ndim != 4:
        raise ValueError(f"{name} must be (N, C, H, W), got shape {tuple(stack.shape)}")
    if stack.dtype not in _DTYPE:
        raise TypeError(f"{name} dtype {stack.dtype} unsupported (uint8, uint16 codes or float32 pixels)")
    if stack.shape[0] > 0 and not stack[0].is_contiguous():
        raise ValueError(f"every image of {name} must be contiguous (C, H, W)")


def _default_max_code(t: torch.Tensor, max_code):
    if t.dtype != torch.float32 and max_code is None:
        return 255.0 if t.dtype == torch.uint8 else 65535.0
    return max_code


def _explicit_std(std: torch.Tensor, stack: torch.Tensor, name: str = "stack"):
    _require_device(std, "std")
    if std.shape != stack.shape:
        raise ValueError(f"std shape != {name} shape")
    return std.to(torch.float32).contiguous()


def _checked_out(out, shape, dtype, device, dtype_name=None):
    if out is None:
        return torch.empty(shape, dtype=dtype, device=device)
    _require_device(out, "out")
    if tuple(out.shape) != shape or out.dtype != dtype or out.device != device or not out.is_contiguous():
        raise ValueError(f"out must be a contiguous {dtype_name or dtype} tensor of shape {shape} on {device}")
    return out


def _icrf_struct(lut: Optional[torch.Tensor], interp, channels):
    if lut is None:
        return nv.Icrf(lut_dev=None, n_points=0, interp=nv.INTERP_NONE), None
    _require_device(lut, "lut")
    if lut.ndim != 2 or lut.shape[0] != channels:
        raise ValueError(f"lut must be (C={channels}, L), got {tuple(lut.shape)}")
    if interp not in _INTERP or interp is None:
        raise ValueError(f"Unknown interpolation mode {interp}")
    lut_c = lut.detach().to(torch.float32).contiguous()
    return nv.Icrf(lut_dev=lut_c.data_ptr(), n_points=lut_c.shape[1], interp=_INTERP[interp]), lut_c


class MergeState:

    def __init__(self, shape, device, with_variance: bool):
        self.mean = torch.empty(shape, dtype=torch.float64, device=device)
        self.sumw = torch.empty(shape, dtype=torch.float32, device=device)
        self.var = torch.empty(shape, dtype=torch.float32, device=device) if with_variance else None
        self.batches = 0


def _merge_setup(stack, layout, out_layout, state, finalize, has_std, mean_dtype, reference_order, flags, what):
    if state is None or state.batches == 0:
        flags |= nv.MERGE_FIRST_BATCH
    if finalize:
        flags |= nv.MERGE_FINALIZE
    if reference_order is not None:
        flags |= nv.MERGE_REFERENCE_ORDER if reference_order else nv.MERGE_CLOSED_FORM
    if mean_dtype == torch.float32:
        flags |= nv.MERGE_MEAN_OUT_F32
    elif mean_dtype != torch.float64:
        raise TypeError("mean_dtype must be float64 (reference) or float32")
    out_shape = _out_shape(stack, layout, out_layout)
    if out_layout == "input":
        flags |= nv.MERGE_OUT_AS_INPUT
    if state is None and not finalize:
        raise ValueError(f"a non-final {what} needs a MergeState")
    if state is not None and has_std and state.var is None:
        raise ValueError("MergeState was created without a variance buffer")
    if state is not None and tuple(state.mean.shape) != out_shape:
        raise ValueError(f"MergeState has shape {tuple(state.mean.shape)}, this merge needs {out_shape}")
    mean_out = torch.empty(out_shape, dtype=mean_dtype, device=stack.device) if finalize else None
    std_out = torch.empty(out_shape, dtype=torch.float32, device=stack.device) if (finalize and has_std) else None
    return flags, out_shape, mean_out, std_out


def hdr_merge_batch(stack: torch.Tensor, exposures: torch.Tensor, *, lut: Optional[torch.Tensor] = None,
                    interp: Optional[str] = "linear", gaussian_weight: bool = True,
                    std: Optional[torch.Tensor] = None, std_mode: str = "none", std_value: float = 0.0,
                    max_code: Optional[float] = None, state: Optional[MergeState] = None, finalize: bool = True,
                    tile: Optional[TileGeometry] = None, mean_dtype: torch.dtype = torch.float64, layout: str = "nchw",
                    force_f64_moments: bool = False, reference_order: Optional[bool] = None, out_layout: str = "planar"):
    _check_stack(stack)
    b = stack.shape[0]
    c, h, w = _chw(stack, layout)
    dev = stack.device
    if b < 1:
        raise ValueError("empty batch")
    if std is not None:
        std_mode = "explicit"
        _require_device(std, "std")
        if std.shape != stack.shape or std.dtype != torch.float32 or std.stride() != stack.stride():
            if std.shape != stack.shape:
                raise ValueError(f"std shape {tuple(std.shape)} != stack shape {tuple(stack.shape)}")
            std = std.to(torch.float32).contiguous()
            if std.stride() != stack.stride():
                stack = stack.contiguous()
    if std_mode not in _STD:
        raise ValueError(f"unknown std_mode {std_mode}")
    max_code = _default_max_code(stack, max_code)
    if exposures.is_cuda or dev.type != "cuda":
        exposure_dev = exposures.to(device=dev, dtype=torch.float64).contiguous()
    else:
        exposure_dev = exposures.to(torch.float64).contiguous().pin_memory().to(dev, non_blocking=True)
    if exposure_dev.numel() != b:
        raise ValueError(f"{exposure_dev.numel()} exposure times for a batch of {b}")
    icrf, lut_keep = _icrf_struct(lut, interp, c)
    geom = _geometry(stack, tile, layout)
    flags, _, mean_out, std_out = _merge_setup(stack, layout, out_layout, state, finalize, std_mode != "none", mean_dtype,
                                               reference_order, nv.MERGE_F64_MOMENTS if force_f64_moments else 0, "batch")
    with torch.cuda.device(dev):
        rc = nv.load().ct_hdr_merge_batch(
            _ptr(stack), _DTYPE[stack.dtype], float(max_code or 1.0), b, ctypes.byref(geom), _ptr(std), _STD[std_mode],
            float(std_value), _ptr(exposure_dev), ctypes.byref(icrf), nv.WEIGHT_GAUSS if gaussian_weight else nv.WEIGHT_NONE,
            _ptr(state.mean) if state else None, _ptr(state.sumw) if state else None,
            _ptr(state.var) if (state and state.var is not None) else None, _ptr(mean_out), _ptr(std_out), flags,
            _stream(dev))
    nv.check(rc, "ct_hdr_merge_batch")
    del lut_keep
    if state is not None:
        state.batches += 1
    return (mean_out, std_out) if finalize else None


MAX_MERGE_BATCHES = 16


def hdr_merge_batches(stacks, exposures, *, lut: Optional[torch.Tensor] = None, interp: Optional[str] = "linear",
                      gaussian_weight: bool = True, stds=None, std_mode: str = "none", std_value: float = 0.0,
                      max_code: Optional[float] = None, state: Optional[MergeState] = None, finalize: bool = True,
                      tile: Optional[TileGeometry] = None, mean_dtype: torch.dtype = torch.float64, layout: str = "nchw",
                      reference_order: Optional[bool] = None, require_one_launch: bool = False, out_layout: str = "planar"):
    k = len(stacks)
    if k == 0 or k != len(exposures) or (stds is not None and len(stds) != k):
        raise ValueError("stacks / exposures / stds must be non-empty lists of equal length")
    if k > MAX_MERGE_BATCHES:
        raise ValueError(f"at most {MAX_MERGE_BATCHES} batches per call")
    if k == 1:
        return hdr_merge_batch(stacks[0], exposures[0], lut=lut, interp=interp, gaussian_weight=gaussian_weight,
                               std=None if stds is None else stds[0], std_mode=std_mode, std_value=std_value, max_code=max_code,
                               state=state, finalize=finalize, tile=tile, mean_dtype=mean_dtype, layout=layout,
                               reference_order=reference_order, out_layout=out_layout)
    for t in stacks:
        _check_stack(t)
        if t.dtype != stacks[0].dtype or t.shape[1:] != stacks[0].shape[1:] or t.device != stacks[0].device:
            raise ValueError("all batches of one call must share dtype, image shape and device")
    dev = stacks[0].device
    c, h, w = _chw(stacks[0], layout)
    if stds is not None:
        std_mode = "explicit"
        stds = [sd.to(device=dev, dtype=torch.float32).contiguous() for sd in stds]
        for sd, t in zip(stds, stacks):
            if sd.shape != t.shape:
                raise ValueError(f"std shape {tuple(sd.shape)} != stack shape {tuple(t.shape)}")
    if std_mode not in _STD:
        raise ValueError(f"unknown std_mode {std_mode}")
    stacks = [t.contiguous() for t in stacks]
    max_code = _default_max_code(stacks[0], max_code)
    sizes = [int(t.shape[0]) for t in stacks]
    for e, n in zip(exposures, sizes):
        if e.numel() != n:
            raise ValueError(f"{e.numel()} exposure times for a batch of {n}")
    host_exp = torch.cat([e.detach().to("cpu", torch.float64).reshape(-1) for e in exposures])
    exposure_dev = host_exp.pin_memory().to(dev, non_blocking=True) if dev.type == "cuda" else host_exp
    icrf, lut_keep = _icrf_struct(lut, interp, c)
    geom = _geometry(stacks[0], tile, layout)
    has_std = std_mode != "none"
    flags, out_shape, mean_out, std_out = _merge_setup(stacks[0], layout, out_layout, state, finalize, has_std, mean_dtype,
                                                       reference_order, nv.MERGE_REQUIRE_ONE_LAUNCH if require_one_launch else 0,
                                                       "call")
    if state is None:
        state = MergeState(out_shape, dev, has_std)
    ptr_arr = (ctypes.c_void_p * k)(*[t.data_ptr() for t in stacks])
    std_arr = (ctypes.c_void_p * k)(*[sd.data_ptr() for sd in stds]) if stds is not None else None
    size_arr = (ctypes.c_int32 * k)(*sizes)
    with torch.cuda.device(dev):
        rc = nv.load().ct_hdr_merge_batches(
            ptr_arr, std_arr, size_arr, k, _DTYPE[stacks[0].dtype], float(max_code or 1.0), ctypes.byref(geom), _STD[std_mode],
            float(std_value), _ptr(exposure_dev), ctypes.byref(icrf), nv.WEIGHT_GAUSS if gaussian_weight else nv.WEIGHT_NONE,
            _ptr(state.mean), _ptr(state.sumw), _ptr(state.var) if state.var is not None else None, _ptr(mean_out),
            _ptr(std_out), flags, _stream(dev))
    nv.check(rc, "ct_hdr_merge_batches")
    del lut_keep
    state.batches += k
    return (mean_out, std_out) if finalize else None


def linearize_frames(frames: torch.Tensor, lut: torch.Tensor, interp: str = "linear", *,
                     std: Optional[torch.Tensor] = None, std_mode: str = "none", std_value: float = 0.0,
                     max_code: Optional[float] = None, want_std: bool = True, tile: Optional[TileGeometry] = None,
                     layout: str = "nchw", out=None):
    _check_stack(frames, "frames")
    f = frames.shape[0]
    c, h, w = _chw(frames, layout)
    dev = frames.device
    if std is not None:
        std_mode, std = "explicit", _explicit_std(std, frames, "frames")
    max_code = _default_max_code(frames, max_code)
    icrf, lut_keep = _icrf_struct(lut, interp, c)
    frames = frames.contiguous()
    geom = _geometry(frames, tile, layout)
    if out is None:
        lin = torch.empty((f, c, h, w), dtype=torch.float32, device=dev)
        std_out = torch.empty_like(lin) if want_std else None
    else:
        lin, std_out = out
        for name, t in (("out[0]", lin), ("out[1]", std_out)):
            if t is None:
                continue
            _require_device(t, name)
            if t.dtype != torch.float32 or tuple(t.shape) != (f, c, h, w) or not t.is_contiguous():
                raise ValueError(f"{name} must be a contiguous float32 tensor of shape {(f, c, h, w)}")
        if want_std and std_out is None:
            raise ValueError("want_std needs out[1]")
        if not want_std:
            std_out = None
    with torch.cuda.device(dev):
        rc = nv.load().ct_linearize_std(_ptr(frames), _DTYPE[frames.dtype], float(max_code or 1.0), f, ctypes.byref(geom),
                                        _ptr(std), _STD[std_mode], float(std_value), ctypes.byref(icrf), _ptr(lin),
                                        _ptr(std_out), _stream(dev))
    nv.check(rc, "ct_linearize_std")
    del lut_keep
    return lin, std_out


def icrf_forward(x: torch.Tensor, lut: torch.Tensor, interp: str, tile: Optional[TileGeometry] = None):
    _check_stack(x, "image")
    if x.dtype != torch.float32:
        raise TypeError("icrf_forward expects float32 pixel values")
    x = x.contiguous()
    icrf, lut_keep = _icrf_struct(lut, interp, x.shape[1])
    geom = _geometry(x, tile)
    out = torch.empty_like(x)
    with torch.cuda.device(x.device):
        rc = nv.load().ct_linearize_fwd(_ptr(x), x.shape[0], ctypes.byref(geom), ctypes.byref(icrf), _ptr(out),
                                        _stream(x.device))
    nv.check(rc, "ct_linearize_fwd")
    del lut_keep
    return out


def icrf_backward(x: torch.Tensor, grad_out: torch.Tensor, lut: torch.Tensor, interp: str, need_x: bool, need_lut: bool,
                  tile: Optional[TileGeometry] = None):
    _check_stack(x, "image")
    x = x.contiguous()
    grad_out = grad_out.to(torch.float32).contiguous()
    icrf, lut_keep = _icrf_struct(lut, interp, x.shape[1])
    geom = _geometry(x, tile)
    gx = torch.empty_like(x) if need_x else None
    gl = torch.zeros((x.shape[1], lut.shape[1]), dtype=torch.float32, device=x.device) if need_lut else None
    with torch.cuda.device(x.device):
        rc = nv.load().ct_linearize_bwd(_ptr(x), _ptr(grad_out), x.shape[0], ctypes.byref(geom), ctypes.byref(icrf),
                                        _ptr(gx), _ptr(gl), _stream(x.device))
    nv.check(rc, "ct_linearize_bwd")
    del lut_keep
    return gx, gl


def _pair_params(lower, upper, use_relative, use_unc_weight, std_mode, std_value, weight_scale=10.0, pair_band=0):
    return nv.PairParams(lower=float(lower), upper=float(upper), weight_scale=float(weight_scale),
                         use_relative=int(bool(use_relative)), use_uncertainty_weighting=int(bool(use_unc_weight)),
                         std_mode=_STD[std_mode], std_value=float(std_value), pair_band=int(pair_band))


class PairList:

    def __init__(self, i_idx: torch.Tensor, j_idx: torch.Tensor, ratio: torch.Tensor, n_images: int, device):
        i_cpu, j_cpu = i_idx.to("cpu", torch.int64), j_idx.to("cpu", torch.int64)
        self.n_pairs, self.n_images = int(i_cpu.numel()), int(n_images)
        self.i = i_cpu.to(torch.int32).to(device)
        self.j = j_cpu.to(torch.int32).to(device)
        self.ratio = ratio.to("cpu", torch.float64).to(device)
        distance = j_cpu - i_cpu
        self.band = int(distance.max()) if self.n_pairs and int(distance.min()) > 0 else 0
        p_idx = torch.arange(self.n_pairs, dtype=torch.int64)
        owner = torch.cat([i_cpu, j_cpu])
        partner = torch.cat([j_cpu, i_cpu])
        code = torch.cat([p_idx, ~p_idx])
        order = torch.argsort(owner * max(self.n_pairs, 1) + torch.cat([p_idx, p_idx]), stable=True)
        counts = torch.bincount(owner, minlength=n_images) if self.n_pairs else torch.zeros(n_images, dtype=torch.int64)
        offsets = torch.zeros(n_images + 1, dtype=torch.int64)
        offsets[1:] = torch.cumsum(counts[:n_images], dim=0)
        samples, codes = partner[order], code[order]
        self.part_off = offsets.to(torch.int32).to(device)
        self.part_sample = (samples if self.n_pairs else torch.zeros(1, dtype=torch.int64)).to(torch.int32).to(device)
        self.part_pair = (codes if self.n_pairs else torch.zeros(1, dtype=torch.int64)).to(torch.int32).to(device)
        self._workspace = {}

    def workspace(self, channels: int) -> torch.Tensor:
        ws = self._workspace.get(channels)
        if ws is None:
            nbytes = int(nv.load().ct_pair_residual_bwd_workspace(self.n_images, self.n_pairs, channels))
            ws = torch.empty(max(nbytes, 32), dtype=torch.uint8, device=self.i.device)
            self._workspace[channels] = ws
        return ws


def pair_residual_sums(stack: torch.Tensor, pairs: PairList, *, lut: Optional[torch.Tensor], interp: Optional[str],
                       lower: float, upper: float, use_relative: bool, use_unc_weight: bool,
                       std: Optional[torch.Tensor] = None, std_mode: str = "none", std_value: float = 0.0,
                       max_code: Optional[float] = None, level: int = 1, tile: Optional[TileGeometry] = None,
                       center: Optional[torch.Tensor] = None, layout: str = "nchw"):
    _check_stack(stack)
    n = stack.shape[0]
    c, _, _ = _chw(stack, layout)
    dev = stack.device
    if n != pairs.n_images:
        raise ValueError(f"pair list was built for {pairs.n_images} images, stack has {n}")
    if std is not None:
        std_mode, std = "explicit", _explicit_std(std, stack)
        stack = stack.contiguous()
    max_code = _default_max_code(stack, max_code)
    icrf, lut_keep = _icrf_struct(lut, interp, c)
    geom = _geometry(stack, tile, layout)
    prm = _pair_params(lower, upper, use_relative, use_unc_weight, std_mode, std_value)
    sums = torch.zeros((pairs.n_pairs, c, 5), dtype=torch.float64, device=dev)
    if center is not None:
        center = center.to(device=dev, dtype=torch.float64).contiguous()
        if center.shape != (pairs.n_pairs, c):
            raise ValueError(f"center must be (P={pairs.n_pairs}, C={c})")
    if pairs.n_pairs:
        with torch.cuda.device(dev):
            rc = nv.load().ct_pair_residual_fwd(_ptr(stack), _DTYPE[stack.dtype], float(max_code or 1.0), n,
                                                ctypes.byref(geom), _ptr(std), ctypes.byref(icrf), _ptr(pairs.i),
                                                _ptr(pairs.j), _ptr(pairs.ratio), pairs.n_pairs, ctypes.byref(prm),
                                                int(level), _ptr(center), _ptr(sums), _stream(dev))
        nv.check(rc, "ct_pair_residual_fwd")
    del lut_keep
    return sums


def pair_residual_lut_grad(stack: torch.Tensor, pairs: PairList, coef: torch.Tensor, *, lut: torch.Tensor, interp: str,
                           lower: float, upper: float, use_relative: bool, max_code: Optional[float] = None,
                           tile: Optional[TileGeometry] = None, use_unc_weight: bool = False,
                           std: Optional[torch.Tensor] = None, std_mode: str = "none", std_value: float = 0.0,
                           smean: Optional[torch.Tensor] = None, lane_kernel: bool = True, layout: str = "nchw"):
    _check_stack(stack)
    n = stack.shape[0]
    c, _, _ = _chw(stack, layout)
    dev = stack.device
    if std is not None:
        std_mode = "explicit"
        std = std.to(device=dev, dtype=torch.float32).contiguous()
        stack = stack.contiguous()
    if not use_unc_weight:
        std, std_mode = None, "none"
    max_code = _default_max_code(stack, max_code)
    icrf, lut_keep = _icrf_struct(lut, interp, c)
    geom = _geometry(stack, tile, layout)
    prm = _pair_params(lower, upper, use_relative, use_unc_weight, std_mode, std_value,
                       pair_band=pairs.band if lane_kernel else 0)
    if std_mode != "none":
        if smean is None:
            raise ValueError("the uncertainty-weighted backward needs the forward's spatial means")
        smean = smean.to(device=dev, dtype=torch.float64).contiguous()
    else:
        smean = None
    coef = coef.to(device=dev, dtype=torch.float64).contiguous()
    if coef.shape != (pairs.n_pairs, c):
        raise ValueError(f"coef must be (P={pairs.n_pairs}, C={c}), got {tuple(coef.shape)}")
    grad = torch.zeros((c, lut.shape[1]), dtype=torch.float64, device=dev)
    if pairs.n_pairs:
        ws = pairs.workspace(c)
        with torch.cuda.device(dev):
            rc = nv.load().ct_pair_residual_bwd(_ptr(stack), _DTYPE[stack.dtype], float(max_code or 1.0), n,
                                                ctypes.byref(geom), _ptr(std), ctypes.byref(icrf), _ptr(pairs.ratio),
                                                pairs.n_pairs, _ptr(pairs.part_off), _ptr(pairs.part_sample),
                                                _ptr(pairs.part_pair), ctypes.byref(prm), _ptr(coef), _ptr(smean),
                                                _ptr(grad), _ptr(ws), ws.numel(), _stream(dev))
        nv.check(rc, "ct_pair_residual_bwd")
    del lut_keep
    return grad


def band_stats(mean: torch.Tensor, std: Optional[torch.Tensor] = None) -> torch.Tensor:
    _require_device(mean, "mean")
    if mean.dtype != torch.float64 or mean.dim() != 3:
        raise ValueError("mean must be a (C, H, W) float64 device tensor")
    mean = mean.contiguous()
    c = mean.shape[0]
    plane = mean.shape[1] * mean.shape[2]
    if std is not None:
        _require_device(std, "std")
        if std.dtype != torch.float32 or std.shape != mean.shape:
            raise ValueError("std must be float32 with the mean's shape")
        std = std.contiguous()
    lib = nv.load()
    ws_bytes = int(lib.ct_band_stats_workspace(c))
    ws = torch.empty((ws_bytes // 8,), dtype=torch.float64, device=mean.device)
    out = torch.empty((6, c), dtype=torch.float64, device=mean.device)
    with torch.cuda.device(mean.device):
        rc = lib.ct_band_stats(_ptr(mean), _ptr(std), c, plane, _ptr(ws), ws_bytes, _ptr(out), _stream(mean.device))
    nv.check(rc, "ct_band_stats")
    return out


def flatfield_correct(value: torch.Tensor, var_or_std: Optional[torch.Tensor], flat: torch.Tensor,
                      flat_std: Optional[torch.Tensor], *, input_is_variance: bool, through_mean: bool,
                      global_pixels: Optional[int] = None, reduce=None):
    _require_device(value, "value")
    flat = flat.to(device=value.device, dtype=torch.float32).contiguous()
    if flat.ndim == 4:
        flat = flat[0]
    c, h, w = flat.shape
    plane = h * w
    if tuple(value.shape[-3:]) != (c, h, w):
        raise ValueError(f"flat field {tuple(flat.shape)} does not match the image {tuple(value.shape)}")
    if not value.is_contiguous():
        raise ValueError("value must be contiguous")
    frames = 1 if value.ndim == 3 else value.shape[0]
    is_f64 = value.dtype == torch.float64
    if value.dtype not in (torch.float64, torch.float32):
        raise TypeError("value must be float32 or float64")
    if flat_std is not None:
        flat_std = flat_std.to(device=value.device, dtype=torch.float32).contiguous()
        if flat_std.ndim == 4:
            flat_std = flat_std[0]
    dev = value.device
    sums = torch.zeros((c, 2), dtype=torch.float64, device=dev)
    with torch.cuda.device(dev):
        rc = nv.load().ct_flatfield_sums(_ptr(value) if (through_mean and frames == 1) else None, int(is_f64), _ptr(flat),
                                         c, plane, _ptr(sums), _stream(dev))
    nv.check(rc, "ct_flatfield_sums")
    if reduce is not None:
        reduce(sums)
    n_px = float(global_pixels if global_pixels is not None else plane)
    flat_mean = (sums[:, 0] / n_px).to(torch.float32).contiguous()
    through = (sums[:, 1] / n_px).contiguous() if through_mean else None
    with torch.cuda.device(dev):
        rc = nv.load().ct_flatfield_apply(_ptr(value), int(is_f64), frames, _ptr(var_or_std), int(input_is_variance),
                                          _ptr(flat), _ptr(flat_std), _ptr(flat_mean), _ptr(through), c, plane, _stream(dev))
    nv.check(rc, "ct_flatfield_apply")
    return value, var_or_std


def dark_field_blur(stack: torch.Tensor, dark: torch.Tensor, dark_std: Optional[torch.Tensor], *,
                    std: Optional[torch.Tensor] = None, std_mode: str = "none", std_value: float = 0.0,
                    max_code: Optional[float] = None, tile: Optional[TileGeometry] = None,
                    halo: Optional[torch.Tensor] = None, threshold: float = 0.05, alpha: float = 50.0):
    _check_stack(stack)
    b, c, h, w = stack.shape
    dev = stack.device
    if std is not None:
        std_mode, std = "explicit", _explicit_std(std, stack)
    stack = stack.contiguous()
    max_code = _default_max_code(stack, max_code)
    dark = dark.to(device=dev, dtype=torch.float32).contiguous()
    if dark.ndim != 4 or dark.shape[0] not in (1, b) or tuple(dark.shape[1:]) != (c, h, w):
        raise ValueError(f"mask_map batch dimension must be 1 or {b}, got shape {tuple(dark.shape)}")
    if dark_std is not None:
        dark_std = dark_std.to(device=dev, dtype=torch.float32).contiguous()
        if dark_std.shape != dark.shape:
            raise ValueError("dark_std shape != dark shape")
        if dark.shape[0] == 1 and b > 1:
            raise NotImplementedError(
                "one shared dark field for several frames with its uncertainty: the reference sums the dark-field gradient "
                "over the frames before squaring, which the per-frame effective sigma of this kernel cannot express; pass "
                "one (matched) dark field per frame, as get_matching_artefact_images does")
    if halo is not None:
        halo = halo.to(device=dev, dtype=stack.dtype).contiguous()
        if tuple(halo.shape) != (b, c, 2, w):
            raise ValueError(f"halo must be (B, C, 2, W) = {(b, c, 2, w)}, got {tuple(halo.shape)}")
    geom = _geometry(stack, tile)
    xb = torch.empty((b, c, h, w), dtype=torch.float32, device=dev)
    sig = torch.empty_like(xb) if dark_std is not None else None
    with torch.cuda.device(dev):
        rc = nv.load().ct_dark_field_blur(_ptr(stack), _DTYPE[stack.dtype], float(max_code or 1.0), b, ctypes.byref(geom),
                                          _ptr(halo), _ptr(std), _STD[std_mode], float(std_value), _ptr(dark),
                                          _ptr(dark_std), dark.shape[0], float(threshold), float(alpha), _ptr(xb), _ptr(sig),
                                          _stream(dev))
    nv.check(rc, "ct_dark_field_blur")
    return xb, sig


def downscaled_shape(shape, step: int, layout: str = "nchw"):
    b, d1, d2, d3 = shape
    if layout == "nchw":
        return b, d1, -(-d2 // step), -(-d3 // step)
    return b, -(-d1 // step), -(-d2 // step), d3


def strided_downscale(stack: torch.Tensor, step: int, layout: str = "nchw", out: Optional[torch.Tensor] = None):
    _check_ingest_stack(stack, layout, for_ingest=False)
    if isinstance(step, bool) or not isinstance(step, int) or step < 1:
        raise ValueError(f"step must be an int >= 1, got {step!r}")
    shape = downscaled_shape(stack.shape, step, layout)
    if step == 1 and out is None:
        return stack
    out = _checked_out(out, shape, stack.dtype, stack.device)
    if step == 1:
        alias = torch.int16 if stack.dtype == torch.uint16 else stack.dtype
        out.view(alias).copy_(stack.view(alias))
        return out
    stack = stack.contiguous()
    if out.numel() == 0:
        return out
    if layout == "nchw":
        planes, h, w, pixel_elems = stack.shape[0] * stack.shape[1], stack.shape[2], stack.shape[3], 1
    else:
        planes, h, w, pixel_elems = stack.shape[0], stack.shape[1], stack.shape[2], stack.shape[3]
    with torch.cuda.device(stack.device):
        rc = nv.load().ct_strided_downscale(_ptr(stack), _ptr(out), stack.element_size(), planes, h, w, pixel_elems, step,
                                            _stream(stack.device))
    nv.check(rc, "ct_strided_downscale")
    return out


_EXPORT_DTYPES = (torch.float32, torch.float64)


def export_shape(shape):
    if len(shape) == 2:
        return tuple(shape)
    if len(shape) == 3:
        return shape[1], shape[2], shape[0]
    if len(shape) == 4:
        return shape[0], shape[2], shape[3], shape[1]
    raise ValueError(f"x must be (H, W), (C, H, W) or (F, C, H, W), got shape {tuple(shape)}")


def export_cv(x: torch.Tensor, dtype: Optional[torch.dtype] = None, out: Optional[torch.Tensor] = None):
    _require_device(x, "x")
    if x.dtype not in _EXPORT_DTYPES:
        raise TypeError(f"x dtype {x.dtype} unsupported (float32 or float64)")
    if dtype is None:
        dtype = x.dtype
    if dtype not in _EXPORT_DTYPES:
        raise TypeError(f"dtype {dtype} unsupported (torch.float32, torch.float64 or None)")
    shape = export_shape(tuple(x.shape))
    if not x.is_contiguous():
        raise ValueError("x must be contiguous")
    out = _checked_out(out, shape, dtype, x.device)
    if out.numel() == 0:
        return out
    if x.ndim == 2:
        images, channels, plane = 1, 1, x.numel()
    else:
        channels, plane = x.shape[-3], x.shape[-2] * x.shape[-1]
        images = x.shape[0] if x.ndim == 4 else 1
    with torch.cuda.device(x.device):
        rc = nv.load().ct_export_cv(_ptr(x), int(x.dtype == torch.float64), _ptr(out), int(dtype == torch.float64), images,
                                    channels, plane, int(channels == 3), _stream(x.device))
    nv.check(rc, "ct_export_cv")
    return out


def ingest_shape(shape, layout: str = "nchw"):
    b, d1, d2, d3 = shape
    return (b, d1, d2, d3) if layout == "nchw" else (b, d3, d1, d2)


def _number(v, what):
    if isinstance(v, bool) or not isinstance(v, (int, float)):
        raise TypeError(f"{what} must be an int or a float, got {v!r}")
    return float(v)


def _ingest_stages(stages, channels: int, data: bool = False, limit: int = nv.INGEST_MAX_STAGES):
    stages = list(stages)
    if len(stages) > limit:
        raise ValueError(f"at most {limit} stages, got {len(stages)}")
    kinds = ("affine", "clamp", "affine_data") if data else ("affine", "clamp")
    arr = (nv.IngestStage * max(len(stages), 1))()
    n_data = 0
    for k, st in enumerate(stages):
        if not isinstance(st, (tuple, list)) or not st or st[0] not in kinds:
            extra = " or ('affine_data', mul, add)" if data else ""
            raise ValueError(f"stage {k}: expected ('affine', sub, div, mul, add) or ('clamp', pairs){extra}, got {st!r}")
        if st[0] == "affine_data":
            n_data += 1
            if len(st) != 3 or n_data > 1:
                raise ValueError(f"stage {k}: one ('affine_data', mul, add) stage with two constants at most")
            arr[k].kind, arr[k].mul, arr[k].add = nv.INGEST_AFFINE_DATA, _number(st[1], f"stage {k}"), _number(st[2], f"stage {k}")
            continue
        if st[0] == "affine":
            if len(st) != 5:
                raise ValueError(f"stage {k}: ('affine', sub, div, mul, add) takes four constants")
            sub, div, mul, add = (_number(v, f"stage {k}") for v in st[1:])
            arr[k].kind, arr[k].sub, arr[k].div, arr[k].mul, arr[k].add = nv.INGEST_AFFINE, sub, div, mul, add
            if arr[k].div == 0.0:
                raise ValueError("Normalization range is zero (min == max); cannot normalize.")
            continue
        if len(st) != 2 or not isinstance(st[1], (tuple, list)):
            raise ValueError(f"stage {k}: ('clamp', pairs) takes a list of (lo, hi) pairs")
        pairs = list(st[1])
        if len(pairs) not in (1, channels) or (len(pairs) > 1 and channels > nv.INGEST_MAX_CHANNELS):
            raise ValueError(f"stage {k}: expected 1 or {channels} min/max pairs (at most {nv.INGEST_MAX_CHANNELS} "
                             f"channels with one pair each), got {len(pairs)}")
        if len(pairs) == 1:
            pairs = pairs * nv.INGEST_MAX_CHANNELS
        pairs += [pairs[-1]] * (nv.INGEST_MAX_CHANNELS - len(pairs))
        arr[k].kind = nv.INGEST_CLAMP
        for c, pair in enumerate(pairs):
            if not isinstance(pair, (tuple, list)) or len(pair) != 2:
                raise ValueError(f"stage {k}: a clamp pair is (lo, hi), got {pair!r}")
            arr[k].lo[c], arr[k].hi[c] = _number(pair[0], f"stage {k}"), _number(pair[1], f"stage {k}")
    return arr, len(stages)


def _check_ingest_stack(stack: torch.Tensor, layout: str, for_ingest: bool = True):
    _require_device(stack, "stack")
    if stack.ndim != 4:
        raise ValueError(f"stack must be 4-dimensional, got shape {tuple(stack.shape)}")
    if stack.dtype not in _DTYPE:
        raise TypeError(f"stack dtype {stack.dtype} unsupported (uint8, uint16 codes or float32 pixels)")
    if layout not in _LAYOUT:
        raise ValueError(f"unknown layout {layout!r} (nchw, nhwc, nhwc_bgr)")
    if not for_ingest:
        return
    if layout != "nchw" and stack.shape[3] != 3:
        raise ValueError(f"layout {layout!r} takes (B, H, W, 3) frames, got shape {tuple(stack.shape)}")
    if not stack.is_contiguous():
        raise ValueError("stack must be contiguous")


def _check_consts(consts, device):
    _require_device(consts, "consts")
    if consts.dtype != torch.float32 or tuple(consts.shape) != (4,) or consts.device != device or not consts.is_contiguous():
        raise ValueError(f"consts must be the 4-element float32 tensor of ingest_extrema on {device}")


def ingest_transform(stack: torch.Tensor, stages, layout: str = "nchw", out: Optional[torch.Tensor] = None,
                     consts: Optional[torch.Tensor] = None):
    _check_ingest_stack(stack, layout)
    shape = ingest_shape(tuple(stack.shape), layout)
    arr, n_stages = _ingest_stages(stages, shape[1], data=consts is not None)
    if consts is not None:
        _check_consts(consts, stack.device)
    out = _checked_out(out, shape, torch.float32, stack.device, "float32")
    if out.numel() == 0:
        return out
    with torch.cuda.device(stack.device):
        if consts is None:
            rc = nv.load().ct_ingest_transform(_ptr(stack), _DTYPE[stack.dtype], _LAYOUT[layout], shape[0], shape[1],
                                               shape[2] * shape[3], arr, n_stages, _ptr(out), _stream(stack.device))
        else:
            rc = nv.load().ct_ingest_transform_data(_ptr(stack), _DTYPE[stack.dtype], _LAYOUT[layout], shape[0], shape[1],
                                                    shape[2] * shape[3], arr, n_stages, _ptr(out), _ptr(consts),
                                                    _stream(stack.device))
    nv.check(rc, "ct_ingest_transform" if consts is None else "ct_ingest_transform_data")
    return out


def linearize_ingest_frames(frames: torch.Tensor, stages, lut: Optional[torch.Tensor], interp: Optional[str] = "linear", *,
                            std: Optional[torch.Tensor] = None, std_mode: str = "none", std_value: float = 0.0,
                            want_std: bool = True, tile: Optional[TileGeometry] = None, layout: str = "nchw", out=None):
    _check_ingest_stack(frames, layout)
    shape = ingest_shape(tuple(frames.shape), layout)
    f, c, h, w = shape
    dev = frames.device
    arr, n_stages = _ingest_stages(stages, c)
    if std is not None:
        std_mode = "explicit"
        _require_device(std, "std")
        if std.dtype != torch.float32 or tuple(std.shape) != shape or std.device != dev:
            raise ValueError(f"std must be a float32 tensor of shape {shape} (planar, like the outputs) on {dev}")
        std = std.contiguous()
    if std_mode not in _STD:
        raise ValueError(f"unknown std_mode {std_mode}")
    icrf, lut_keep = _icrf_struct(lut, interp, c)
    hg, r0 = (h, 0) if tile is None else (tile.h_global, tile.row_offset)
    if r0 < 0 or r0 + h > hg:
        raise ValueError(f"tile rows [{r0}, {r0 + h}) do not fit a global height of {hg}")
    geom = nv.Geometry(channels=c, h_tile=h, width=w, h_global=hg, row_offset=r0, image_stride=c * h * w, layout=_LAYOUT[layout])
    if out is None:
        lin = torch.empty(shape, dtype=torch.float32, device=dev)
        std_out = torch.empty_like(lin) if want_std else None
    else:
        lin, std_out = out
        for name, t in (("out[0]", lin), ("out[1]", std_out)):
            if t is None:
                continue
            _require_device(t, name)
            if t.dtype != torch.float32 or tuple(t.shape) != shape or not t.is_contiguous():
                raise ValueError(f"{name} must be a contiguous float32 tensor of shape {shape}")
        if lin is None:
            raise ValueError("out[0] is required")
        if want_std and std_out is None:
            raise ValueError("want_std needs out[1]")
        if not want_std:
            std_out = None
    if frames.numel() == 0:
        return lin, std_out
    with torch.cuda.device(dev):
        rc = nv.load().ct_linearize_ingest(_ptr(frames), _DTYPE[frames.dtype], f, ctypes.byref(geom), arr, n_stages, _ptr(std),
                                           _STD[std_mode], float(std_value), ctypes.byref(icrf), _ptr(lin), _ptr(std_out),
                                           _stream(dev))
    nv.check(rc, "ct_linearize_ingest")
    del lut_keep
    return lin, std_out


ZERO_RANGE = "Normalization range is zero (min == max); cannot normalize."


def ingest_extrema(stack: torch.Tensor, prefix_stages=(), layout: str = "nchw", min_val=None, max_val=None):
    _check_ingest_stack(stack, layout)
    if min_val is not None and max_val is not None:
        raise ValueError("min_val and max_val are both given: nothing depends on the data (use ingest_transform)")
    shape = ingest_shape(tuple(stack.shape), layout)
    arr, n_prefix = _ingest_stages(prefix_stages, shape[1], limit=nv.EXTREMA_MAX_PREFIX)
    from_data = (nv.EXTREMA_MIN if min_val is None else 0) | (nv.EXTREMA_MAX if max_val is None else 0)
    fixed_min = 0.0 if min_val is None else _number(min_val, "min_val")
    fixed_max = 0.0 if max_val is None else _number(max_val, "max_val")
    if stack.numel() == 0:
        raise RuntimeError("ingest_extrema: the stack is empty (the extrema of an empty tensor are undefined)")
    lib = nv.load()
    ws_bytes = int(lib.ct_ingest_extrema_workspace())
    ws = torch.empty((ws_bytes // 4,), dtype=torch.float32, device=stack.device)
    consts = torch.empty((4,), dtype=torch.float32, device=stack.device)
    with torch.cuda.device(stack.device):
        rc = lib.ct_ingest_extrema(_ptr(stack), _DTYPE[stack.dtype], _LAYOUT[layout], shape[0], shape[1], shape[2] * shape[3],
                                   arr, n_prefix, from_data, fixed_min, fixed_max, _ptr(ws), ws_bytes, _ptr(consts),
                                   _stream(stack.device))
    nv.check(rc, "ct_ingest_extrema")
    return consts


def data_stage_prefix(stages):
    stages = list(stages)
    at = [k for k, st in enumerate(stages) if isinstance(st, (tuple, list)) and st and st[0] == "affine_data"]
    if len(at) != 1:
        raise ValueError(f"stages must hold exactly one ('affine_data', mul, add) stage, got {len(at)}")
    return stages[:at[0]]


def check_ingest_consts(consts: torch.Tensor):
    if float(consts.cpu()[1]) == 0.0:
        raise ValueError(ZERO_RANGE)


def ingest_transform_data(stack: torch.Tensor, stages, layout: str = "nchw", min_val=None, max_val=None, check: bool = True,
                          out: Optional[torch.Tensor] = None):
    consts = ingest_extrema(stack, data_stage_prefix(stages), layout, min_val, max_val)
    out = ingest_transform(stack, stages, layout, out=out, consts=consts)
    if not check:
        return out, consts
    check_ingest_consts(consts)
    return out


def video_stats_batch(frames: torch.Tensor, mean_state: torch.Tensor, m2_state: torch.Tensor, frames_before: int, *,
                      lut: Optional[torch.Tensor] = None, interp: Optional[str] = None,
                      max_code: Optional[float] = None, tile: Optional[TileGeometry] = None, layout: str = "nchw"):
    _check_stack(frames, "frames")
    b = frames.shape[0]
    c, h, w = _chw(frames, layout)
    dev = frames.device
    frames = frames.contiguous()
    max_code = _default_max_code(frames, max_code)
    for name, t in (("mean_state", mean_state), ("m2_state", m2_state)):
        _require_device(t, name)
        if t.dtype != torch.float32 or tuple(t.shape) != (c, h, w) or not t.is_contiguous():
            raise ValueError(f"{name} must be a contiguous float32 (C,H,W) tensor")
    icrf, lut_keep = _icrf_struct(lut, interp, c)
    geom = _geometry(frames, tile, layout)
    with torch.cuda.device(dev):
        rc = nv.load().ct_video_stats_batch(_ptr(frames), _DTYPE[frames.dtype], float(max_code or 1.0), b,
                                            ctypes.byref(geom), ctypes.byref(icrf), float(frames_before),
                                            _ptr(mean_state), _ptr(m2_state), _stream(dev))
    nv.check(rc, "ct_video_stats_batch")
    del lut_keep
```

include/clair_hip.h:

```cpp
#ifndef CLAIR_HIP_H
#define CLAIR_HIP_H

#include <stdint.h>

#ifdef __cplusplus
extern "C" {
#endif

#define CT_ABI_VERSION 3

#define CT_OK 0
#define CT_ERR_INVALID_ARGUMENT (-1)
#define CT_ERR_UNSUPPORTED (-2)
#define CT_ERR_LAUNCH (-3)
#define CT_ERR_NO_GRADIENT_PATH (-4)
#define CT_ERR_TOO_LARGE (-5)

#define CT_DTYPE_U8 0
#define CT_DTYPE_U16 1
#define CT_DTYPE_F32 2

#define CT_INTERP_LOOKUP 0
#define CT_INTERP_LINEAR 1
#define CT_INTERP_CATMULL 2
#define CT_INTERP_NONE 3

#define CT_STD_NONE 0
#define CT_STD_CONSTANT 1
#define CT_STD_MULTIPLIER 2
#define CT_STD_EXPLICIT 3

#define CT_WEIGHT_NONE 0
#define CT_WEIGHT_GAUSS 1

#define CT_MERGE_FIRST_BATCH 1u
#define CT_MERGE_FINALIZE 2u
#define CT_MERGE_MEAN_OUT_F32 4u
#define CT_MERGE_F64_MOMENTS 8u
#define CT_MERGE_REFERENCE_ORDER 16u
#define CT_MERGE_CLOSED_FORM 32u
#define CT_MERGE_REQUIRE_ONE_LAUNCH 128u
#define CT_MERGE_STD_HINT 64u
#define CT_MERGE_OUT_AS_INPUT 256u

#define CT_LAYOUT_NCHW 0
#define CT_LAYOUT_NHWC 1
#define CT_LAYOUT_NHWC_BGR 2

typedef struct ct_geometry {
    int32_t channels;
    int64_t h_tile;
    int64_t width;
    int64_t h_global;
    int64_t row_offset;
    int64_t image_stride;
    int32_t layout;
} ct_geometry;

typedef struct ct_icrf {
    const float *lut_dev;
    int32_t n_points;
    int32_t interp;
} ct_icrf;

int ct_abi_version(void);
const char *ct_error_string(int code);

int ct_hdr_merge_batch(const void *stack_dev, int32_t dtype, float max_code, int32_t batch, const ct_geometry *geom,
                       const float *std_dev, int32_t std_mode, float std_value, const double *exposure_dev,
                       const ct_icrf *icrf, int32_t weight_mode, double *mean_state_dev, float *sumw_state_dev,
                       float *var_state_dev, void *mean_out_dev, float *std_out_dev, uint32_t flags, void *stream);

int ct_hdr_merge_batches(const void *const *stack_devs, const float *const *std_devs, const int32_t *batch_sizes,
                         int32_t n_batches, int32_t dtype, float max_code, const ct_geometry *geom, int32_t std_mode,
                         float std_value, const double *exposure_dev, const ct_icrf *icrf, int32_t weight_mode,
                         double *mean_state_dev, float *sumw_state_dev, float *var_state_dev, void *mean_out_dev,
                         float *std_out_dev, uint32_t flags, void *stream);

int ct_norm_constants(float max_code, float *hi, float *lo);
int ct_index_constants(float max_code, int n_points, float *hi, float *lo);
int ct_pivot_index_constants(float max_code, int n_points, uint32_t *index_mul, float *step);
int ct_pivot_floor_constants(float max_code, int n_points, float *rcp_step);
int ct_pivot_interval_constants(float max_code, int n_points, int lookup, int dtype_max, float *scale);

const char *ct_hdr_merge_kernel_name(int32_t dtype, float max_code, int32_t interp, int32_t n_points, uint32_t flags);

void ct_merge_set_retry_counter(unsigned long long *counter_dev);

int ct_linearize_std(const void *frames_dev, int32_t dtype, float max_code, int64_t n_frames, const ct_geometry *geom,
                     const float *std_dev, int32_t std_mode, float std_value, const ct_icrf *icrf, float *lin_out_dev,
                     float *std_out_dev, void *stream);

int ct_linearize_fwd(const float *x_dev, int64_t n_images, const ct_geometry *geom, const ct_icrf *icrf,
                     float *out_dev, void *stream);
int ct_linearize_bwd(const float *x_dev, const float *grad_out_dev, int64_t n_images, const ct_geometry *geom,
                     const ct_icrf *icrf, float *grad_x_dev, float *lut_grad_dev, void *stream);

typedef struct ct_pair_params {
    float lower, upper;
    float weight_scale;
    int32_t use_relative;
    int32_t use_uncertainty_weighting;
    int32_t std_mode;
    float std_value;
    int32_t pair_band;
} ct_pair_params;

int ct_pair_residual_fwd(const void *stack_dev, int32_t dtype, float max_code, int32_t n_images,
                         const ct_geometry *geom, const float *std_dev, const ct_icrf *icrf, const int32_t *i_idx_dev,
                         const int32_t *j_idx_dev, const double *ratio_dev, int32_t n_pairs,
                         const ct_pair_params *params, int32_t level, const double *center_dev, double *sums_dev,
                         void *stream);

int64_t ct_pair_residual_bwd_workspace(int32_t n_images, int32_t n_pairs, int32_t channels);
int ct_pair_residual_bwd(const void *stack_dev, int32_t dtype, float max_code, int32_t n_images,
                         const ct_geometry *geom, const float *std_dev, const ct_icrf *icrf, const double *ratio_dev,
                         int32_t n_pairs, const int32_t *partner_offsets_dev, const int32_t *partner_sample_dev,
                         const int32_t *partner_pair_dev, const ct_pair_params *params, const double *coef_dev,
                         const double *smean_dev, double *lut_grad_dev, void *workspace_dev, int64_t workspace_bytes,
                         void *stream);

int ct_flatfield_sums(const void *value_dev, int32_t value_is_f64, const float *flat_dev, int32_t channels,
                      int64_t plane, double *sums_dev, void *stream);
int ct_flatfield_apply(void *value_dev, int32_t value_is_f64, int64_t n_frames, float *var_or_std_dev,
                       int32_t input_is_variance, const float *flat_dev, const float *flat_std_dev,
                       const float *flat_mean_dev, const double *through_mean_dev, int32_t channels, int64_t plane,
                       void *stream);

int64_t ct_band_stats_workspace(int32_t channels);
int ct_band_stats(const double *mean_dev, const float *std_dev, int32_t channels, int64_t plane, void *workspace_dev,
                  int64_t workspace_bytes, double *out_dev, void *stream);

int ct_dark_field_blur(const void *stack_dev, int32_t dtype, float max_code, int32_t batch, const ct_geometry *geom,
                       const void *halo_dev, const float *std_dev, int32_t std_mode, float std_value,
                       const float *dark_dev, const float *dark_std_dev, int32_t dark_batch, float threshold, float alpha,
                       float *xb_out_dev, float *std_out_dev, void *stream);

int ct_video_stats_batch(const void *frames_dev, int32_t dtype, float max_code, int32_t batch, const ct_geometry *geom,
                         const ct_icrf *icrf, float frames_before, float *mean_state_dev, float *m2_state_dev,
                         void *stream);

int ct_strided_downscale(const void *src_dev, void *dst_dev, int32_t elem_bytes, int64_t n_planes, int64_t h, int64_t w,
                         int32_t pixel_elems, int32_t step, void *stream);

#define CT_INGEST_AFFINE 0
#define CT_INGEST_CLAMP 1
#define CT_INGEST_MAX_STAGES 4
#define CT_INGEST_MAX_CHANNELS 4
typedef struct {
    int32_t kind;
    float sub, div, mul, add;
    float lo[CT_INGEST_MAX_CHANNELS];
    float hi[CT_INGEST_MAX_CHANNELS];
} ct_ingest_stage;
int ct_ingest_transform(const void *src_dev, int32_t dtype, int32_t layout, int64_t n_images, int32_t channels,
                        int64_t plane, const ct_ingest_stage *stages, int32_t n_stages, float *dst_dev, void *stream);

#define CT_INGEST_AFFINE_DATA 2
#define CT_EXTREMA_MIN 1
#define CT_EXTREMA_MAX 2
#define CT_EXTREMA_MAX_PREFIX 3
int64_t ct_ingest_extrema_workspace(void);
int ct_ingest_extrema(const void *src_dev, int32_t dtype, int32_t layout, int64_t n_images, int32_t channels, int64_t plane,
                      const ct_ingest_stage *prefix, int32_t n_prefix, int32_t from_data, float fixed_min, float fixed_max,
                      void *workspace_dev, int64_t workspace_bytes, float *consts_dev, void *stream);
int ct_ingest_transform_data(const void *src_dev, int32_t dtype, int32_t layout, int64_t n_images, int32_t channels,
                             int64_t plane, const ct_ingest_stage *stages, int32_t n_stages, float *dst_dev,
                             const float *consts_dev, void *stream);

int ct_linearize_ingest(const void *frames_dev, int32_t dtype, int64_t n_frames, const ct_geometry *geom,
                        const ct_ingest_stage *stages, int32_t n_stages, const float *std_dev, int32_t std_mode,
                        float std_value, const ct_icrf *icrf, float *lin_out_dev, float *std_out_dev, void *stream);

int ct_export_cv(const void *src_dev, int32_t src_is_f64, void *dst_dev, int32_t dst_is_f64, int64_t n_images,
                 int32_t channels, int64_t plane, int32_t reverse_channels, void *stream);

#ifdef __cplusplus
}
#endif
#endif
```

Measured before the change: 19670 MPix/s.

## Replace per-pixel Gaussian exp with piecewise-linear weight table fused into LUT gather

Adds a host-side search for a subdivision of the ICRF interval grid on which the Gaussian weight is piecewise linear within one float32 ulp. The pivot merge kernel then reads the weight slope and intercept together with the LUT entry in a single 16-byte LDS gather instead of computing exp2 per code. This targets transcendental ALU cost in the merge inner loop. In exchange it uses more LDS per workgroup, adds new kernel template variants with 1024-thread blocks, and makes weights approximate to within a relative bound. An exp_weight flag keeps the old path available.

```diff
diff --git a/clair_torch_amd/_native.py b/clair_torch_amd/_native.py
--- a/clair_torch_amd/_native.py
+++ b/clair_torch_amd/_native.py
@@ -10,6 +10,8 @@
 LAYOUT_NCHW, LAYOUT_NHWC, LAYOUT_NHWC_BGR = 0, 1, 2
 MERGE_FIRST_BATCH, MERGE_FINALIZE, MERGE_MEAN_OUT_F32, MERGE_F64_MOMENTS = 1, 2, 4, 8
 MERGE_REFERENCE_ORDER, MERGE_CLOSED_FORM, MERGE_STD_HINT, MERGE_REQUIRE_ONE_LAUNCH, MERGE_OUT_AS_INPUT = 16, 32, 64, 128, 256
+MERGE_EXP_WEIGHT = 512
+WTAB_REL_BOUND = 2.0 ** -23
 INGEST_AFFINE, INGEST_CLAMP, INGEST_MAX_STAGES, INGEST_MAX_CHANNELS = 0, 1, 4, 4
 INGEST_AFFINE_DATA, EXTREMA_MIN, EXTREMA_MAX, EXTREMA_MAX_PREFIX = 2, 1, 2, 3
 ERR_NO_GRADIENT_PATH = -4
@@ -21,7 +23,7 @@
            "ct_merge_set_retry_counter", "ct_norm_constants", "ct_index_constants", "ct_pivot_index_constants",
            "ct_pivot_floor_constants", "ct_pivot_interval_constants", "ct_band_stats", "ct_band_stats_workspace",
            "ct_strided_downscale", "ct_export_cv", "ct_ingest_transform", "ct_ingest_extrema_workspace", "ct_ingest_extrema",
-           "ct_ingest_transform_data", "ct_linearize_ingest")
+           "ct_ingest_transform_data", "ct_linearize_ingest", "ct_merge_weight_table", "ct_hdr_merge_kernel_name_ex")
 
 
 class Geometry(ctypes.Structure):
@@ -92,6 +94,10 @@
     lib.ct_pair_residual_bwd_workspace.argtypes = [i32, i32, i32]
     lib.ct_hdr_merge_kernel_name.restype = ctypes.c_char_p
     lib.ct_hdr_merge_kernel_name.argtypes = [i32, f32, i32, i32, u32]
+    lib.ct_hdr_merge_kernel_name_ex.restype = ctypes.c_char_p
+    lib.ct_hdr_merge_kernel_name_ex.argtypes = [i32, f32, i32, i32, i32, i32, i32, u32]
+    lib.ct_merge_weight_table.restype = i32
+    lib.ct_merge_weight_table.argtypes = [i32, f32, i32, i32, f32, ctypes.POINTER(i32), ctypes.POINTER(f32), vp, vp]
     lib.ct_merge_set_retry_counter.restype = None
     lib.ct_merge_set_retry_counter.argtypes = [vp]
     lib.ct_flatfield_sums.restype = i32
diff --git a/clair_torch_amd/build.py b/clair_torch_amd/build.py
--- a/clair_torch_amd/build.py
+++ b/clair_torch_amd/build.py
@@ -9,7 +9,7 @@
 LIB_DIR = os.path.join(HERE, "lib")
 LIB_PATH = os.path.join(LIB_DIR, "libclair_hip.so")
 OBJ_DIR = os.path.join(LIB_DIR, "obj")
-SOURCES = ["ct_merge.hip", "ct_merge_multi.hip", "ct_merge_exact.hip", "ct_linearize.hip", "ct_pairs.hip", "ct_flatfield.hip", "ct_stats.hip", "ct_darkfield.hip", "ct_bandstats.hip",
+SOURCES = ["ct_merge.hip", "ct_merge_multi.hip", "ct_merge_wtab.hip", "ct_merge_exact.hip", "ct_linearize.hip", "ct_pairs.hip", "ct_flatfield.hip", "ct_stats.hip", "ct_darkfield.hip", "ct_bandstats.hip",
            "ct_downscale.hip", "ct_export.hip", "ct_ingest.hip", "ct_extrema.hip", "ct_linearize_ingest.hip", "ct_api.cpp"]
 HEADERS = ["ct_device.hpp", "ct_merge.hpp", "ct_merge_pivot.hpp", "ct_ingest_stages.hpp", os.path.join("..", "..", "include", "clair_hip.h")]
 FLAGS = ["--offload-arch=gfx950", "-O3", "-std=c++17", "-fPIC", "-ffp-contract=off",
diff --git a/clair_torch_amd/csrc/ct_api.cpp b/clair_torch_amd/csrc/ct_api.cpp
--- a/clair_torch_amd/csrc/ct_api.cpp
+++ b/clair_torch_amd/csrc/ct_api.cpp
@@ -219,3 +219,114 @@
     *scale = found;
     return rc;
 }
+
+static const size_t kWtabTableBudget = 160 * 1024 - 48 * 1024 - 8 * 1024;
+
+extern "C" int ct_merge_weight_table(int32_t dtype, float max_code, int32_t n_points, int32_t channels, float weight_scale,
+                                     int32_t *subdiv, float *index_rcp, float *weights_out, int32_t *entries_out)
+{
+    struct Entry { int32_t dtype, n_points, channels; float max_code, weight_scale; int rc; int32_t subdiv; float rcp; };
+    static std::mutex mu;
+    static Entry cache[8];
+    static int used = 0, next = 0;
+    if (dtype != CT_DTYPE_U8 && dtype != CT_DTYPE_U16) return CT_ERR_UNSUPPORTED;
+    const int dtype_max = dtype == CT_DTYPE_U8 ? 255 : 65535;
+    if (max_code != (float)dtype_max || n_points < 2 || channels < 1 || !(weight_scale > 0.0f) || !(weight_scale < 1e6f) || !subdiv || !index_rcp)
+        return CT_ERR_UNSUPPORTED;
+    std::lock_guard<std::mutex> lock(mu);
+    const bool want_tables = weights_out || entries_out;
+    if (!want_tables)
+        for (int k = 0; k < used; ++k)
+            if (cache[k].dtype == dtype && cache[k].n_points == n_points && cache[k].channels == channels && cache[k].max_code == max_code &&
+                cache[k].weight_scale == weight_scale) {
+                *subdiv = cache[k].subdiv;
+                *index_rcp = cache[k].rcp;
+                return cache[k].rc;
+            }
+    int rc = CT_ERR_UNSUPPORTED;
+    int32_t found_R = 0;
+    float found_rcp = 0.0f;
+    float lut_scale = 0.0f;
+    const int top = n_points - 1;
+    if (ct_pivot_interval_constants(max_code, n_points, 0, dtype_max, &lut_scale) == CT_OK) {
+        int le = 0;
+        const uint64_t LM = (uint64_t)ldexp(frexp((double)lut_scale, &le), 24);
+        const int lshift = 24 - le;
+        volatile float kk = sqrtf(weight_scale * 1.4426950408889634f);
+        volatile float inv_max = (float)(1.0 / (double)max_code);
+        volatile float dk_mul = kk * inv_max, dk_add = -0.5f * kk;
+        float *w = new float[dtype_max + 1];
+        int32_t *sub = new int32_t[dtype_max + 1];
+        for (int u = 0; u <= dtype_max; ++u) {
+            volatile float dk = fmaf((float)u, dk_mul, dk_add);
+            volatile float sq = dk * dk;
+            w[u] = exp2f(-sq);
+        }
+        static const int kSubdivs[6] = {1, 2, 4, 8, 12, 16};
+        for (int ri = 0; ri < 6 && rc != CT_OK; ++ri) {
+            const int R = kSubdivs[ri];
+            const int64_t last = (int64_t)R * top;
+            if ((size_t)channels * (size_t)(last + 1) * 16 > kWtabTableBudget) break;
+            if (R > 1 && (double)R * top > (double)max_code) break;
+            const double want = (double)last / (double)max_code;
+            float cand[4];
+            cand[0] = (float)want;
+            if ((double)cand[0] < want) cand[0] = nextafterf(cand[0], INFINITY);
+            cand[1] = nextafterf(cand[0], INFINITY);
+            cand[2] = nextafterf(cand[0], 0.0f);
+            cand[3] = nextafterf(cand[2], 0.0f);
+            for (int c = 0; c < 4 && rc != CT_OK; ++c) {
+                const float r = cand[c];
+                if (!((double)dtype_max * (double)r < 4194304.0)) continue;
+                int e = 0;
+                const uint64_t M = (uint64_t)ldexp(frexp((double)r, &e), 24);
+                const int shift = 24 - e;
+                if (shift < 0 || shift >= 63 || lshift < 0 || lshift >= 63) continue;
+                bool ok = true;
+                for (int u = 0; ok && u <= dtype_max; ++u) {
+                    const uint64_t j = ((uint64_t)u * M) >> shift;
+                    uint64_t li = ((uint64_t)u * LM) >> lshift;
+                    if (li > (uint64_t)top) li = (uint64_t)top;
+                    ok = j <= (uint64_t)last && j / (uint64_t)R == li;
+                    sub[u] = (int32_t)j;
+                }
+                for (int u0 = 0; ok && u0 <= dtype_max;) {
+                    int u1 = u0;
+                    while (u1 < dtype_max && sub[u1 + 1] == sub[u0]) ++u1;
+                    const double ws = u1 > u0 ? ((double)w[u1] - (double)w[u0]) / (double)(u1 - u0) : 0.0;
+                    const float wsf = (float)ws;
+                    double lo = (double)w[u0] - (double)wsf * (double)u0, hi = lo;
+                    for (int u = u0 + 1; u <= u1; ++u) {
+                        const double res = (double)w[u] - (double)wsf * (double)u;
+                        lo = fmin(lo, res);
+                        hi = fmax(hi, res);
+                    }
+                    const float waf = (float)(0.5 * (lo + hi));
+                    for (int u = u0; ok && u <= u1; ++u) {
+                        const float wt = fmaf(wsf, (float)u, waf);
+                        const double err = fabs((double)wt - (double)w[u]);
+                        ok = err <= (double)CT_WTAB_REL_BOUND * (double)w[u];
+                        if (weights_out) weights_out[u] = wt;
+                    }
+                    u0 = u1 + 1;
+                }
+                if (ok) {
+                    rc = CT_OK;
+                    found_R = R;
+                    found_rcp = r;
+                    if (entries_out)
+                        for (int u = 0; u <= dtype_max; ++u) entries_out[u] = sub[u];
+                }
+            }
+        }
+        delete[] w;
+        delete[] sub;
+    }
+    if (!want_tables) {
+        Entry &slot = cache[used < 8 ? used++ : (next++ % 8)];
+        slot = Entry{dtype, n_points, channels, max_code, weight_scale, rc, found_R, found_rcp};
+    }
+    *subdiv = found_R;
+    *index_rcp = found_rcp;
+    return rc;
+}
diff --git a/clair_torch_amd/csrc/ct_merge.hip b/clair_torch_amd/csrc/ct_merge.hip
--- a/clair_torch_amd/csrc/ct_merge.hip
+++ b/clair_torch_amd/csrc/ct_merge.hip
@@ -349,10 +349,7 @@
         size_t lds = pivot_lds_bytes(a, x, INTERP);
         x.rgb252 = 0;
         if constexpr (V == 4) {
-            auto aligned16 = [](const void *p) { return (reinterpret_cast<uintptr_t>(p) % 16) == 0; };
-            if (a.tile.layout != CT_LAYOUT_NCHW && !(a.flags & CT_MERGE_OUT_AS_INPUT) && a.channels == 3 && a.tile.plane_local % 4 == 0 && !a.mean_state &&
-                (a.flags & CT_MERGE_FINALIZE) && !(a.flags & CT_MERGE_MEAN_OUT_F32) && a.q_begin == 0 &&
-                a.q_count == 3u * a.tile.plane_local && aligned16(a.mean_out) && aligned16(a.std_out)) {
+            if (pivot_rgb252_applies(a)) {
                 x.rgb252 = 1;
                 lds = (lds + 15) & ~(size_t)15;
                 x.stage_off = (uint32_t)lds;
@@ -445,10 +442,16 @@
             const uint32_t q_pv = packets_aligned(a, sizeof(T), kPivotV, false) ? (Q / kPivotV) * kPivotV : 0;
             a.q_begin = 0;
             a.q_count = q_pv;
-            if (q_pv) rc = dispatch_pivot<T, kPivotV>(a, *pivot, interp, weight_mode, std_mode, pivot_clamp, s);
+            constexpr int dtype = sizeof(T) == 1 ? CT_DTYPE_U8 : CT_DTYPE_U16;
+            const bool wtab = pivot->wtab_subdiv != 0;
+            if (q_pv)
+                rc = wtab ? merge_pivot_wtab(a, *pivot, dtype, kPivotV, std_mode, false, s)
+                          : dispatch_pivot<T, kPivotV>(a, *pivot, interp, weight_mode, std_mode, pivot_clamp, s);
             a.q_begin = q_pv;
             a.q_count = Q - q_pv;
-            if (rc == CT_OK && q_pv < Q) rc = dispatch_pivot<T, 1>(a, *pivot, interp, weight_mode, std_mode, pivot_clamp, s);
+            if (rc == CT_OK && q_pv < Q)
+                rc = wtab ? merge_pivot_wtab(a, *pivot, dtype, 1, std_mode, false, s)
+                          : dispatch_pivot<T, 1>(a, *pivot, interp, weight_mode, std_mode, pivot_clamp, s);
             return rc;
         }
     }
@@ -467,6 +470,9 @@
 extern "C" int ct_norm_constants(float max_code, float *hi, float *lo);
 extern "C" int ct_index_constants(float max_code, int n_points, float *hi, float *lo);
 extern "C" int ct_pivot_interval_constants(float max_code, int n_points, int lookup, int dtype_max, float *scale);
+extern "C" int ct_merge_weight_table(int32_t dtype, float max_code, int32_t n_points, int32_t channels, float weight_scale,
+                                     int32_t *subdiv, float *index_rcp, float *weights_out, int32_t *entries_out);
+static constexpr float kGaussWeightScale = 30.0f;
 
 static unsigned long long *g_merge_retry_counter = nullptr;
 extern "C" void ct_merge_set_retry_counter(unsigned long long *counter_dev) { g_merge_retry_counter = counter_dev; }
@@ -477,9 +483,10 @@
     Generic
 };
 
-static MergeRoute merge_route(int32_t dtype, float max_code, int interp, int n_points, int std_mode, uint32_t flags,
-                              ct::PivotArgs *px, bool *clamp)
-{
+static MergeRoute merge_route(int32_t dtype, float max_code, int interp, int n_points, int channels, int weight_mode, int std_mode,
+                              uint32_t flags, ct::PivotArgs *px, bool *clamp)
+{
+    px->wtab_subdiv = 0;
     if (flags & CT_MERGE_REFERENCE_ORDER) return MergeRoute::ReferenceOrder;
     if ((interp == CT_INTERP_CATMULL || interp == CT_INTERP_LOOKUP) && std_mode != CT_STD_NONE &&
         !(flags & (CT_MERGE_CLOSED_FORM | CT_MERGE_F64_MOMENTS)))
@@ -501,18 +508,34 @@
     px->step = (float)((double)max_code / (double)(n_points - 1));
     px->n_entries = lookup ? 2u * (uint32_t)n_points : (uint32_t)n_points;
     px->tf_max = ct::kFloorMagic + (float)(lookup ? 2 * (n_points - 1) : n_points - 1);
+    if (interp == CT_INTERP_LINEAR && weight_mode == CT_WEIGHT_GAUSS && std_mode != CT_STD_EXPLICIT && !*clamp && !(flags & CT_MERGE_EXP_WEIGHT)) {
+        int32_t subdiv = 0;
+        float rcp = 0.0f;
+        if (ct_merge_weight_table(dtype, max_code, n_points, channels, kGaussWeightScale, &subdiv, &rcp, nullptr, nullptr) == CT_OK) {
+            px->wtab_subdiv = (uint32_t)subdiv;
+            px->wtab_entries = (uint32_t)subdiv * (uint32_t)(n_points - 1) + 1u;
+            px->wtab_rcp = rcp;
+        }
+    }
     return MergeRoute::Pivot;
 }
 
-extern "C" const char *ct_hdr_merge_kernel_name(int32_t dtype, float max_code, int32_t interp, int32_t n_points,
-                                                uint32_t flags)
+extern "C" const char *ct_hdr_merge_kernel_name_ex(int32_t dtype, float max_code, int32_t interp, int32_t n_points, int32_t channels,
+                                                   int32_t weight_mode, int32_t std_mode, uint32_t flags)
 {
     ct::PivotArgs px{};
     bool clamp = false;
-    switch (merge_route(dtype, max_code, interp, n_points, (flags & CT_MERGE_STD_HINT) ? CT_STD_CONSTANT : CT_STD_NONE, flags, &px, &clamp)) {
+    switch (merge_route(dtype, max_code, interp, n_points, channels, weight_mode, std_mode, flags, &px, &clamp)) {
         case MergeRoute::ReferenceOrder:
             return "ct::merge_reference_order_kernel (the reference's float32 autograd order, two passes, float64 exp and divisions)";
         case MergeRoute::Pivot:
+            if (px.wtab_subdiv)
+                return (flags & CT_MERGE_FIRST_BATCH)
+                           ? "ct::merge_pivot_kernel, fused weight table (float32 moments about a per-pixel pivot, Gaussian weight read "
+                             "with the LUT entry in one 16-byte gather, persistent 1024-thread workgroups, 4 codes per thread "
+                             "through typed buffer loads, first batch)"
+                           : "ct::merge_pivot_kernel, fused weight table (float32 moments about the running mean, Gaussian weight "
+                             "read with the LUT entry in one 16-byte gather, persistent 1024-thread workgroups, streaming state)";
             return (flags & CT_MERGE_FIRST_BATCH)
                        ? "ct::merge_pivot_kernel (float32 moments about a per-pixel pivot, persistent workgroups, 4 codes per "
                          "thread through typed buffer loads, 7 wavefronts per SIMD, first batch)"
@@ -525,6 +548,13 @@
                                      : "ct::merge_kernel (float64 moments, integer codes)";
     return dtype == CT_DTYPE_F32 ? "ct::merge_kernel (float32 moments about a per-pixel pivot, float32 pixels, 4 per thread)"
                                  : "ct::merge_kernel (float32 moments about a per-pixel pivot, integer codes through the float LUT coordinate)";
+}
+
+extern "C" const char *ct_hdr_merge_kernel_name(int32_t dtype, float max_code, int32_t interp, int32_t n_points,
+                                                uint32_t flags)
+{
+    return ct_hdr_merge_kernel_name_ex(dtype, max_code, interp, n_points, 3, CT_WEIGHT_GAUSS,
+                                       (flags & CT_MERGE_STD_HINT) ? CT_STD_CONSTANT : CT_STD_NONE, flags | CT_MERGE_EXP_WEIGHT);
 }
 
 struct MergeCall {
@@ -591,7 +621,7 @@
     a.channels = geom->channels;
     a.n_points = c.icrf->interp == CT_INTERP_NONE ? 2 : c.icrf->n_points;
     a.std_value = c.std_value;
-    a.weight_scale = 30.0f;
+    a.weight_scale = kGaussWeightScale;
     a.inv_max_code = 1.0f;
     a.flags = c.flags;
     return a;
@@ -614,7 +644,7 @@
     hipStream_t s = static_cast<hipStream_t>(stream);
     PivotArgs px{};
     bool clamp = false;
-    const MergeRoute route = merge_route(dtype, max_code, interp, a.n_points, std_mode, flags, &px, &clamp);
+    const MergeRoute route = merge_route(dtype, max_code, interp, a.n_points, a.channels, weight_mode, std_mode, flags, &px, &clamp);
     if (dtype != CT_DTYPE_F32 && ct_norm_constants(max_code, &a.norm.hi, &a.norm.lo) != CT_OK) return CT_ERR_UNSUPPORTED;
     if (route == MergeRoute::ReferenceOrder) return merge_reference_order(a, dtype, Ql, interp, weight_mode, std_mode, s);
     if (dtype == CT_DTYPE_F32) return merge_typed<float>(a, Ql, interp, weight_mode, std_mode, s, false);
@@ -651,7 +681,7 @@
     MergeArgs a = fill_merge_args(c, stack_devs[0], std_mode == CT_STD_EXPLICIT ? std_devs[0] : nullptr, (int32_t)total);
     PivotArgs px{};
     bool clamp = false;
-    const MergeRoute route = merge_route(dtype, max_code, interp, a.n_points, std_mode, flags, &px, &clamp);
+    const MergeRoute route = merge_route(dtype, max_code, interp, a.n_points, a.channels, weight_mode, std_mode, flags, &px, &clamp);
 
     if (route == MergeRoute::ReferenceOrder && valid == CT_OK && n_batches >= 2 && n_batches <= kMaxMergeBatches && total <= 65536 &&
         (dtype == CT_DTYPE_U8 || dtype == CT_DTYPE_U16 || dtype == CT_DTYPE_F32)) {
@@ -689,6 +719,7 @@
             px.batch_ptr[b] = stack_devs[b];
             px.std_ptr[b] = std_mode == CT_STD_EXPLICIT ? std_devs[b] : nullptr;
         }
+        if (px.wtab_subdiv) return merge_pivot_wtab(a, px, dtype, kPivotV, std_mode, true, s);
         return merge_pivot_multi(a, px, dtype, clamp, interp, weight_mode, std_mode, s);
     }
     if (flags & CT_MERGE_REQUIRE_ONE_LAUNCH) return CT_ERR_UNSUPPORTED;
diff --git a/clair_torch_amd/csrc/ct_merge_pivot.hpp b/clair_torch_amd/csrc/ct_merge_pivot.hpp
--- a/clair_torch_amd/csrc/ct_merge_pivot.hpp
+++ b/clair_torch_amd/csrc/ct_merge_pivot.hpp
@@ -69,6 +69,9 @@
     const float *std_ptr[16];
     int32_t rgb252;
     uint32_t stage_off;
+    uint32_t wtab_subdiv;
+    uint32_t wtab_entries;
+    float wtab_rcp;
 };
 constexpr int kMaxMultiBatches = 16;
 constexpr int kPivotV = 4;
@@ -76,13 +79,21 @@
 constexpr int kPivotDepth = 2;
 constexpr float kRoughLimit = 64.0f;
 
+constexpr int kWtabBlock = 1024;
+#ifndef CT_WTAB_DEPTH
+#define CT_WTAB_DEPTH 3
+#endif
+constexpr int kWtabDepth = CT_WTAB_DEPTH;
 
 constexpr int kRgb252Waves = 6;
-template <typename T, int V, int INTERP, int WEIGHT, int STD, bool FIRST, bool CLAMP = false, bool MULTI = false, bool RGB252 = false>
-__global__ __launch_bounds__(kBlock)
-__attribute__((amdgpu_waves_per_eu(FIRST && V <= 4 && STD != CT_STD_EXPLICIT ? (RGB252 ? kRgb252Waves : 7) : 4, 8)))
+template <typename T, int V, int INTERP, int WEIGHT, int STD, bool FIRST, bool CLAMP = false, bool MULTI = false, bool RGB252 = false,
+          bool WTAB = false, int BLOCK = kBlock, int DEPTH = kPivotDepth>
+__global__ __launch_bounds__(BLOCK)
+__attribute__((amdgpu_waves_per_eu(WTAB ? 4 : FIRST && V <= 4 && STD != CT_STD_EXPLICIT ? (RGB252 ? kRgb252Waves : 7) : 4, 8)))
 void merge_pivot_kernel(const MergeArgs a, const PivotArgs x)
 {
+    static_assert(!WTAB || (INTERP == CT_INTERP_LINEAR && WEIGHT == CT_WEIGHT_GAUSS && STD != CT_STD_EXPLICIT && !CLAMP),
+                  "WTAB: LINEAR, Gaussian weights, full-range codes");
     static_assert(!MULTI || !FIRST, "MULTI carries state");
     static_assert(!RGB252 || (V == 4 && FIRST && !MULTI), "RGB252: single-batch packets");
     extern __shared__ __align__(16) char lds[];
@@ -95,8 +106,7 @@
     using CodePk = Packet<float, V>;
     const int C = a.channels, L = a.n_points, B = a.batch;
     constexpr int kEntryShift = kCat ? 4 : 3;
-    const int E = kLut ? (int)x.n_entries : 0;
-    const int lut_bytes = C * E * (1 << kEntryShift);
+    const int lut_bytes = WTAB ? C * (int)x.wtab_entries * 16 : kLut ? C * (int)x.n_entries * (1 << kEntryShift) : 0;
     float2 *expo = reinterpret_cast<float2 *>(lds + lut_bytes);
     const float kk = sqrtf(a.weight_scale * 1.4426950408889634f);
     const float dk_mul = kk * a.inv_max_code, dk_add = -0.5f * kk;
@@ -106,8 +116,9 @@
 
     bool rough = false;
     if constexpr (kLookup) {
+        const int E = (int)x.n_entries;
         const int total = C * E;
-        for (int k = threadIdx.x; k < total; k += kBlock) {
+        for (int k = threadIdx.x; k < total; k += BLOCK) {
             const int r = k / E, j = k - r * E;
             const int idx = (j + 1) >> 1;
             reinterpret_cast<float2 *>(lds)[k] = make_float2(a.lut[(size_t)r * L + (idx < L ? idx : L - 1)], 0.0f);
@@ -115,7 +126,7 @@
     } else if constexpr (kCat) {
         const int total = C * L;
         const double st = (double)x.step;
-        for (int k = threadIdx.x; k < total; k += kBlock) {
+        for (int k = threadIdx.x; k < total; k += BLOCK) {
             const int r = k / L, i = k - r * L;
             const float *row = a.lut + (size_t)r * L;
             const double p0 = row[i > 0 ? i - 1 : 0], p1 = row[i], p2 = row[i + 1 < L ? i + 1 : L - 1], p3 = row[i + 2 < L ? i + 2 : L - 1];
@@ -126,7 +137,7 @@
         const int total = C * L;
         const double stepd = (double)x.max_code / (double)(L - 1);
         bool viol = false;
-        for (int k = threadIdx.x; k < total; k += kBlock) {
+        for (int k = threadIdx.x; k < total; k += BLOCK) {
             const int r = k / L, i = k - r * L;
             const float *row = a.lut + (size_t)r * L;
             const float g0 = row[i], g1 = row[i + 1 < L ? i + 1 : L - 1];
@@ -135,16 +146,64 @@
             viol |= !(fabsf(A) <= kRoughLimit * fmaxf(fmaxf(fabsf(g0), fabsf(g1)), 1e-30f));
         }
         rough = __syncthreads_or(viol);
-        for (int k = threadIdx.x; k < total; k += kBlock) {
+        for (int k = threadIdx.x; k < total; k += BLOCK) {
             const int r = k / L, i = k - r * L;
             const float *row = a.lut + (size_t)r * L;
             const float g0 = row[i], g1 = row[i + 1 < L ? i + 1 : L - 1];
             const float slope = (g1 - g0) / x.step;
             const float A = (float)((double)g0 - (double)slope * ((double)i * stepd));
-            reinterpret_cast<float2 *>(lds)[k] = make_float2(rough ? g0 : A, slope);
+            if (!WTAB || rough) reinterpret_cast<float2 *>(lds)[k] = make_float2(rough ? g0 : A, slope);
+        }
+        if constexpr (WTAB) {
+            if (!rough) {
+                const int R = (int)x.wtab_subdiv, J = (int)x.wtab_entries;
+                const int cmax = (int)x.max_code;
+                auto sub_of = [&](int c) -> int {
+                    const float cf[1] = {(float)c};
+                    float t[1];
+                    floor_index_bits<1>(cf, x.wtab_rcp, kFloorMagic, t);
+                    return (int)(__float_as_uint(t[0]) - kFloorMagicBits);
+                };
+                auto first_code = [&](int j) -> int {
+                    if (j >= J) return cmax + 1;
+                    int c = (int)((float)j / x.wtab_rcp);
+                    c = c < 0 ? 0 : (c > cmax ? cmax : c);
+                    while (c > 0 && sub_of(c - 1) >= j) --c;
+                    while (c <= cmax && sub_of(c) < j) ++c;
+                    return c;
+                };
+                auto weight_of = [&](int c) -> double {
+                    const float dk = __builtin_fmaf((float)c, dk_mul, dk_add);
+                    return (double)__builtin_amdgcn_exp2f(-dk * dk);
+                };
+                for (int j = threadIdx.x; j < J; j += BLOCK) {
+                    const int c0 = first_code(j), c1 = first_code(j + 1) - 1;
+                    double ws = 0.0, wa = 0.0;
+                    if (c1 >= c0) {
+                        const double w0 = weight_of(c0);
+                        ws = c1 > c0 ? (weight_of(c1) - w0) / (double)(c1 - c0) : 0.0;
+                        const float wsf = (float)ws;
+                        double lo = w0 - (double)wsf * (double)c0, hi = lo;
+                        for (int c = c0 + 1; c <= c1; ++c) {
+                            const double r = weight_of(c) - (double)wsf * (double)c;
+                            lo = fmin(lo, r);
+                            hi = fmax(hi, r);
+                        }
+                        wa = 0.5 * (lo + hi);
+                    }
+                    const int i = j / R;
+                    for (int r = 0; r < C; ++r) {
+                        const float *row = a.lut + (size_t)r * L;
+                        const float g0 = row[i], g1 = row[i + 1 < L ? i + 1 : L - 1];
+                        const float slope = (g1 - g0) / x.step;
+                        const float A = (float)((double)g0 - (double)slope * ((double)i * stepd));
+                        reinterpret_cast<float4 *>(lds)[r * J + j] = make_float4(A, slope, (float)wa, (float)ws);
+                    }
+                }
+            }
         }
     }
-    for (int n = threadIdx.x; n < B; n += kBlock) {
+    for (int n = threadIdx.x; n < B; n += BLOCK) {
         const float it = (float)(1.0 / a.exposure[n]);
         expo[n] = make_float2(it, ce * it);
     }
@@ -159,13 +218,16 @@
     if constexpr (STD == CT_STD_CONSTANT) fsf *= a.std_value;
     if constexpr (STD == CT_STD_MULTIPLIER) fsf *= a.std_value * a.inv_max_code;
     const float sv2 = fsf * fsf;
-    [[maybe_unused]] const float index_rcp = x.index_rcp;
+    const bool wtab = WTAB && !rough;
+    [[maybe_unused]] const float index_rcp = wtab ? x.wtab_rcp : x.index_rcp;
+    const int E = wtab ? (int)x.wtab_entries : kLut ? (int)x.n_entries : 0;
+    [[maybe_unused]] const int entry_shift = wtab ? 4 : kEntryShift;
     [[maybe_unused]] float floor_magic = kFloorMagic;
     asm volatile("" : "+v"(floor_magic));
 
     constexpr bool rgb252 = RGB252;
     for (uint32_t tile = blockIdx.x; tile < x.n_tiles; tile += gridDim.x) {
-        const uint32_t vec = tile * (uint32_t)kBlock + threadIdx.x;
+        const uint32_t vec = tile * (uint32_t)BLOCK + threadIdx.x;
         if (vec * (uint32_t)V >= a.q_count) continue;
         const uint32_t q0 = a.q_begin + vec * (uint32_t)V;
 
@@ -215,7 +277,7 @@
         [[maybe_unused]] uint32_t rowc[V];
         if constexpr (kLut) {
 #pragma unroll
-            for (int e = 0; e < V; ++e) rowc[e] = lds_row_constant<kEntryShift>(row_off[e] << (kEntryShift - 3));
+            for (int e = 0; e < V; ++e) rowc[e] = (uint32_t)(row_off[e] << (entry_shift - 3)) - (kFloorMagicBits << entry_shift);
         }
 
         const uint32_t voff = q0 * (uint32_t)sizeof(T), svoff = q0 * 4u;
@@ -252,7 +314,11 @@
                     if constexpr (CLAMP) o = px > x.max_code ? 0.0f : o;
                     lin = __builtin_fmaf(__builtin_fmaf(__builtin_fmaf(g.w, o, g.z), o, g.y), o, g.x);
                 } else if constexpr (kLut) {
-                    const float2 g = *reinterpret_cast<const float2 *>(lds + lds_entry_address<kEntryShift>(tf[e], rowc[e]));
+                    float2 g;
+                    if (wtab)
+                        g = *reinterpret_cast<const float2 *>(lds + lds_entry_address<4>(tf[e], rowc[e]));
+                    else
+                        g = *reinterpret_cast<const float2 *>(lds + lds_entry_address<kEntryShift>(tf[e], rowc[e]));
                     lin = __builtin_fmaf(g.y, rough ? __builtin_fmaf(tf[e] - floor_magic, -x.step, px) : px, g.x);
                 }
                 p[e] = lin * itp;
@@ -300,6 +366,7 @@
 
             auto run_batch = [&](auto rough_c, auto moments_c) {
             constexpr bool kRough = decltype(rough_c)::value;
+            constexpr bool kTab = WTAB && !kRough;
             constexpr bool kMoments = decltype(moments_c)::value;
             auto reduce = [&](const CodePk &pk, const Packet<float, V> &sp, uint32_t expo_adr) {
                 const float2 ex = *reinterpret_cast<const float2 *>(lds + expo_adr);
@@ -331,18 +398,25 @@
                             gs[e] = __builtin_fmaf(__builtin_fmaf(3.0f * g.w, o, g.z + g.z), o, g.y);
                             if constexpr (CLAMP) gs[e] = above ? 0.0f : gs[e];
                         }
+                    } else if constexpr (kTab) {
+                        typedef float f4 __attribute__((ext_vector_type(4)));
+                        const f4 g = *static_cast<const f4 *>(__builtin_assume_aligned(lds + lds_entry_address<4>(tf[e], rowc[e]), 16));
+                        ga[e] = g.x;
+                        gs[e] = g.y;
+                        wv[e] = __builtin_fmaf(g.w, pxv[e], g.z);
+                        dkv[e] = __builtin_fmaf(pxv[e], dk_mul, dk_add);
                     } else if constexpr (kLut) {
                         const float2 g = *reinterpret_cast<const float2 *>(lds + lds_entry_address(tf[e], rowc[e]));
                         ga[e] = g.x;
                         gs[e] = g.y;
                         if constexpr (kRough) pxl[e] = __builtin_fmaf(tf[e] - floor_magic, -x.step, pxv[e]);
                     }
-                    if constexpr (kGauss) {
+                    if constexpr (kGauss && !kTab) {
                         dkv[e] = __builtin_fmaf(pxv[e], dk_mul, dk_add);
                         wv[e] = __builtin_amdgcn_exp2f(-dkv[e] * dkv[e]);
                     }
                 });
-                if constexpr (kGauss) {
+                if constexpr (kGauss && !kTab) {
 #pragma unroll
                     for (int e = 0; e < V; ++e) asm volatile("" : "+v"(wv[e]));
                 }
@@ -394,18 +468,18 @@
                     sp = load_buffer<Packet<float, V>>(sbase, svoff);
                 }
             };
-            constexpr int kRing = kPivotDepth + 1;
+            constexpr int kRing = DEPTH + 1;
             CodePk ring[kRing];
             Packet<float, V> sring[STD == CT_STD_EXPLICIT ? kRing : 1];
-            static_for<kPivotDepth>([&](auto jc) {
+            static_for<DEPTH>([&](auto jc) {
                 constexpr int j = decltype(jc)::value;
                 fetch(j, ring[j], sring[STD == CT_STD_EXPLICIT ? j : 0]);
             });
             uint32_t expo_adr = (uint32_t)lut_bytes + 8u * (uint32_t)n0;
             for (int n = 0; n < Bb; n += kRing) {
                 static_for<kRing>([&](auto jc) {
-                    constexpr int j = decltype(jc)::value, slot = (j + kPivotDepth) % kRing;
-                    fetch(n + j + kPivotDepth, ring[slot], sring[STD == CT_STD_EXPLICIT ? slot : 0]);
+                    constexpr int j = decltype(jc)::value, slot = (j + DEPTH) % kRing;
+                    fetch(n + j + DEPTH, ring[slot], sring[STD == CT_STD_EXPLICIT ? slot : 0]);
                     if (j == 0 || n + j < Bb) reduce(ring[j], sring[STD == CT_STD_EXPLICIT ? j : 0], expo_adr + 8u * j);
                 });
                 expo_adr += 8u * kRing;
@@ -492,15 +566,15 @@
         }
         if (finalize && rgb252) {
             if constexpr (RGB252) {
-                const uint32_t tile_first = tile * (uint32_t)(kBlock * V);
-                const bool tile_full = tile_first + (uint32_t)(kBlock * V) <= a.q_count;
+                const uint32_t tile_first = tile * (uint32_t)(BLOCK * V);
+                const bool tile_full = tile_first + (uint32_t)(BLOCK * V) <= a.q_count;
                 float sdv[4];
 #pragma unroll
                 for (int e = 0; e < 4; ++e) sdv[e] = kHasStd ? __builtin_amdgcn_sqrtf(var_o[e]) : 0.0f;
                 if (tile_full) {
                     char *stage = lds + x.stage_off;
                     double *sm = reinterpret_cast<double *>(stage);
-                    float *ss = reinterpret_cast<float *>(stage + 8192);
+                    float *ss = reinterpret_cast<float *>(stage + BLOCK * V * 8);
                     typedef double d2 __attribute__((ext_vector_type(2)));
                     typedef float f4 __attribute__((ext_vector_type(4)));
                     __syncthreads();
@@ -512,7 +586,7 @@
                         *reinterpret_cast<f4 *>(ss + 4u * threadIdx.x) = sv;
                     }
                     __syncthreads();
-                    const uint32_t g_first = (tile_first + 11u) / 12u, g_end = (tile_first + (uint32_t)(kBlock * V)) / 12u;
+                    const uint32_t g_first = (tile_first + 11u) / 12u, g_end = (tile_first + (uint32_t)(BLOCK * V)) / 12u;
 #pragma unroll
                     for (int e = 0; e < 4; ++e) {
                         const uint32_t m = q0 + (uint32_t)e - a.q_begin;
@@ -582,32 +656,41 @@
 }
 
 template <typename KernelT>
-static int pivot_blocks_per_cu(KernelT kernel, size_t lds)
+static int pivot_blocks_per_cu(KernelT kernel, size_t lds, int block = kBlock)
 {
     int n = 0;
-    if (hipOccupancyMaxActiveBlocksPerMultiprocessor(&n, kernel, kBlock, lds) != hipSuccess || n < 1) n = 1;
+    if (hipOccupancyMaxActiveBlocksPerMultiprocessor(&n, kernel, block, lds) != hipSuccess || n < 1) n = 1;
     return n < 8 ? n : 8;
 }
 
-template <auto kernel>
+template <auto kernel, int BLOCK = kBlock>
 static int launch_pivot_grid(const MergeArgs &a, const PivotArgs &x, size_t lds, hipStream_t stream)
 {
     static int per_cu = 0;
     static size_t per_cu_lds = 0;
     if (per_cu == 0 || lds > per_cu_lds) {
-        per_cu = pivot_blocks_per_cu(kernel, lds);
+        per_cu = pivot_blocks_per_cu(kernel, lds, BLOCK);
         per_cu_lds = lds;
     }
     uint32_t grid = (uint32_t)(compute_units() * per_cu);
     if (grid > x.n_tiles) grid = x.n_tiles;
-    hipLaunchKernelGGL(kernel, dim3(grid), dim3(kBlock), lds, stream, a, x);
+    hipLaunchKernelGGL(kernel, dim3(grid), dim3(BLOCK), lds, stream, a, x);
     return hipGetLastError() == hipSuccess ? CT_OK : CT_ERR_LAUNCH;
 }
 
-static size_t pivot_lds_bytes(const MergeArgs &a, const PivotArgs &x, int interp)
-{
+static size_t pivot_lds_bytes(const MergeArgs &a, const PivotArgs &x, int interp, bool wtab = false)
+{
+    if (wtab) return (size_t)a.channels * x.wtab_entries * 16 + 2 * sizeof(float) * (size_t)a.batch;
     const size_t table = interp == CT_INTERP_NONE ? 0 : (size_t)a.channels * x.n_entries * (interp == CT_INTERP_CATMULL ? 16 : 8);
     return table + 2 * sizeof(float) * (size_t)a.batch;
+}
+
+static bool pivot_rgb252_applies(const MergeArgs &a)
+{
+    auto aligned16 = [](const void *p) { return (reinterpret_cast<uintptr_t>(p) % 16) == 0; };
+    return a.tile.layout != CT_LAYOUT_NCHW && !(a.flags & CT_MERGE_OUT_AS_INPUT) && a.channels == 3 && a.tile.plane_local % 4 == 0 &&
+           !a.mean_state && (a.flags & CT_MERGE_FINALIZE) && !(a.flags & CT_MERGE_MEAN_OUT_F32) && a.q_begin == 0 &&
+           a.q_count == 3u * a.tile.plane_local && aligned16(a.mean_out) && aligned16(a.std_out);
 }
 
 template <int... VALUES, typename F>
@@ -631,4 +714,7 @@
 int merge_pivot_multi(const MergeArgs &a, const PivotArgs &px, int dtype, bool clamp, int interp, int weight_mode, int std_mode,
                       hipStream_t s);
 
-}
+constexpr size_t kWtabStageBytes = (size_t)kWtabBlock * kPivotV * 12;
+int merge_pivot_wtab(const MergeArgs &a, const PivotArgs &px, int dtype, int v, int std_mode, bool multi, hipStream_t s);
+
+}
diff --git a/clair_torch_amd/csrc/ct_merge_wtab.hip b/clair_torch_amd/csrc/ct_merge_wtab.hip
--- /dev/null
+++ b/clair_torch_amd/csrc/ct_merge_wtab.hip
@@ -0,0 +1,49 @@
+#include "ct_merge_pivot.hpp"
+
+namespace ct {
+
+template <typename T, int V, int STD>
+static int launch_wtab(const MergeArgs &a, PivotArgs x, bool multi, hipStream_t stream)
+{
+    if (a.q_count == 0) return CT_OK;
+    constexpr int I = CT_INTERP_LINEAR, W = CT_WEIGHT_GAUSS, B = kWtabBlock, D = kWtabDepth;
+    x.n_tiles = (a.q_count + (uint32_t)(B * V) - 1) / (uint32_t)(B * V);
+    size_t lds = pivot_lds_bytes(a, x, I, true);
+    x.rgb252 = 0;
+    if constexpr (V == kPivotV) {
+        if (multi) {
+            if (lds > 160 * 1024) return CT_ERR_TOO_LARGE;
+            return launch_pivot_grid<merge_pivot_kernel<T, V, I, W, STD, false, false, true, false, true, B, D>, B>(a, x, lds, stream);
+        }
+        if (pivot_rgb252_applies(a)) {
+            if (!(a.flags & CT_MERGE_FIRST_BATCH)) return CT_ERR_INVALID_ARGUMENT;
+            lds = (lds + 15) & ~(size_t)15;
+            x.rgb252 = 1;
+            x.stage_off = (uint32_t)lds;
+            lds += kWtabStageBytes;
+            if (lds > 160 * 1024) return CT_ERR_TOO_LARGE;
+            return launch_pivot_grid<merge_pivot_kernel<T, V, I, W, STD, true, false, false, true, true, B, D>, B>(a, x, lds, stream);
+        }
+    }
+    if (multi) return CT_ERR_INVALID_ARGUMENT;
+    if (lds > 160 * 1024) return CT_ERR_TOO_LARGE;
+    return (a.flags & CT_MERGE_FIRST_BATCH)
+               ? launch_pivot_grid<merge_pivot_kernel<T, V, I, W, STD, true, false, false, false, true, B, D>, B>(a, x, lds, stream)
+               : launch_pivot_grid<merge_pivot_kernel<T, V, I, W, STD, false, false, false, false, true, B, D>, B>(a, x, lds, stream);
+}
+
+template <typename T>
+static int dispatch_wtab(const MergeArgs &a, const PivotArgs &x, int v, int std_mode, bool multi, hipStream_t s)
+{
+    return with_enum<CT_STD_NONE, CT_STD_CONSTANT, CT_STD_MULTIPLIER>(std_mode, [&](auto S) {
+        return v == 1 ? launch_wtab<T, 1, S>(a, x, multi, s) : launch_wtab<T, kPivotV, S>(a, x, multi, s);
+    });
+}
+
+int merge_pivot_wtab(const MergeArgs &a, const PivotArgs &px, int dtype, int v, int std_mode, bool multi, hipStream_t s)
+{
+    if (!px.wtab_subdiv || (v != 1 && v != kPivotV)) return CT_ERR_INVALID_ARGUMENT;
+    return dtype == CT_DTYPE_U8 ? dispatch_wtab<uint8_t>(a, px, v, std_mode, multi, s) : dispatch_wtab<uint16_t>(a, px, v, std_mode, multi, s);
+}
+
+}
diff --git a/clair_torch_amd/ops.py b/clair_torch_amd/ops.py
--- a/clair_torch_amd/ops.py
+++ b/clair_torch_amd/ops.py
@@ -140,7 +140,8 @@
                     std: Optional[torch.Tensor] = None, std_mode: str = "none", std_value: float = 0.0,
                     max_code: Optional[float] = None, state: Optional[MergeState] = None, finalize: bool = True,
                     tile: Optional[TileGeometry] = None, mean_dtype: torch.dtype = torch.float64, layout: str = "nchw",
-                    force_f64_moments: bool = False, reference_order: Optional[bool] = None, out_layout: str = "planar"):
+                    force_f64_moments: bool = False, reference_order: Optional[bool] = None, out_layout: str = "planar",
+                    exp_weight: bool = False):
     _check_stack(stack)
     b = stack.shape[0]
     c, h, w = _chw(stack, layout)
@@ -168,7 +169,8 @@
     icrf, lut_keep = _icrf_struct(lut, interp, c)
     geom = _geometry(stack, tile, layout)
     flags, _, mean_out, std_out = _merge_setup(stack, layout, out_layout, state, finalize, std_mode != "none", mean_dtype,
-                                               reference_order, nv.MERGE_F64_MOMENTS if force_f64_moments else 0, "batch")
+                                               reference_order, (nv.MERGE_F64_MOMENTS if force_f64_moments else 0) |
+                                               (nv.MERGE_EXP_WEIGHT if exp_weight else 0), "batch")
     with torch.cuda.device(dev):
         rc = nv.load().ct_hdr_merge_batch(
             _ptr(stack), _DTYPE[stack.dtype], float(max_code or 1.0), b, ctypes.byref(geom), _ptr(std), _STD[std_mode],
@@ -190,7 +192,8 @@
                       gaussian_weight: bool = True, stds=None, std_mode: str = "none", std_value: float = 0.0,
                       max_code: Optional[float] = None, state: Optional[MergeState] = None, finalize: bool = True,
                       tile: Optional[TileGeometry] = None, mean_dtype: torch.dtype = torch.float64, layout: str = "nchw",
-                      reference_order: Optional[bool] = None, require_one_launch: bool = False, out_layout: str = "planar"):
+                      reference_order: Optional[bool] = None, require_one_launch: bool = False, out_layout: str = "planar",
+                      exp_weight: bool = False):
     k = len(stacks)
     if k == 0 or k != len(exposures) or (stds is not None and len(stds) != k):
         raise ValueError("stacks / exposures / stds must be non-empty lists of equal length")
@@ -200,7 +203,7 @@
         return hdr_merge_batch(stacks[0], exposures[0], lut=lut, interp=interp, gaussian_weight=gaussian_weight,
                                std=None if stds is None else stds[0], std_mode=std_mode, std_value=std_value, max_code=max_code,
                                state=state, finalize=finalize, tile=tile, mean_dtype=mean_dtype, layout=layout,
-                               reference_order=reference_order, out_layout=out_layout)
+                               reference_order=reference_order, out_layout=out_layout, exp_weight=exp_weight)
     for t in stacks:
         _check_stack(t)
         if t.dtype != stacks[0].dtype or t.shape[1:] != stacks[0].shape[1:] or t.device != stacks[0].device:
@@ -227,8 +230,8 @@
     geom = _geometry(stacks[0], tile, layout)
     has_std = std_mode != "none"
     flags, out_shape, mean_out, std_out = _merge_setup(stacks[0], layout, out_layout, state, finalize, has_std, mean_dtype,
-                                                       reference_order, nv.MERGE_REQUIRE_ONE_LAUNCH if require_one_launch else 0,
-                                                       "call")
+                                                       reference_order, (nv.MERGE_REQUIRE_ONE_LAUNCH if require_one_launch else 0) |
+                                                       (nv.MERGE_EXP_WEIGHT if exp_weight else 0), "call")
     if state is None:
         state = MergeState(out_shape, dev, has_std)
     ptr_arr = (ctypes.c_void_p * k)(*[t.data_ptr() for t in stacks])
diff --git a/include/clair_hip.h b/include/clair_hip.h
--- a/include/clair_hip.h
+++ b/include/clair_hip.h
@@ -42,6 +42,7 @@
 #define CT_MERGE_REQUIRE_ONE_LAUNCH 128u
 #define CT_MERGE_STD_HINT 64u
 #define CT_MERGE_OUT_AS_INPUT 256u
+#define CT_MERGE_EXP_WEIGHT 512u
 
 #define CT_LAYOUT_NCHW 0
 #define CT_LAYOUT_NHWC 1
@@ -83,7 +84,13 @@
 int ct_pivot_floor_constants(float max_code, int n_points, float *rcp_step);
 int ct_pivot_interval_constants(float max_code, int n_points, int lookup, int dtype_max, float *scale);
 
+#define CT_WTAB_REL_BOUND 1.1920929e-7f
+int ct_merge_weight_table(int32_t dtype, float max_code, int32_t n_points, int32_t channels, float weight_scale,
+                          int32_t *subdiv, float *index_rcp, float *weights_out, int32_t *entries_out);
+
 const char *ct_hdr_merge_kernel_name(int32_t dtype, float max_code, int32_t interp, int32_t n_points, uint32_t flags);
+const char *ct_hdr_merge_kernel_name_ex(int32_t dtype, float max_code, int32_t interp, int32_t n_points, int32_t channels,
+                                        int32_t weight_mode, int32_t std_mode, uint32_t flags);
 
 void ct_merge_set_retry_counter(unsigned long long *counter_dev);
 
```

Measured after the change: 19690 MPix/s (median of 4 runs). No clear change (+0.1%).
